# Jack-Tattershall/mujoco-manip

Measured on AMD Instinct MI355X. Metric: env steps/sec (whole node) at 4096 parallel envs; 1/2/4/8 MI355X scaling, higher is better.
Workload: dtype f32

## Files before the change

mujoco_manip_amd/_build.py:

```python
from __future__ import annotations

import os
import subprocess
from concurrent.futures import ThreadPoolExecutor

PKG = os.path.dirname(os.path.abspath(__file__))
CSRC = os.path.join(PKG, "csrc")
LIB = os.path.join(PKG, "libmmx.so")
LIB_PROF = os.path.join(PKG, "libmmx_prof.so")
SOURCES = ["mmx_kernels.hip", "mmx_step_l192.hip", "mmx_render.hip", "mmx_render_lit.hip", "mmx_png.hip",
           "mmx_snapshot.hip", "mmx_mppi.hip", "mmx_policy.hip", "mmx_api.cpp"]
ARCH = os.environ.get("MMX_OFFLOAD_ARCH", "gfx950")
DEVICE_MATH = ["-Xarch_device", "-freciprocal-math", "-Xarch_device", "-fapprox-func",
               "-Xarch_device", "-ffinite-math-only", "-Xarch_device", "-fno-signed-zeros"]
DEVICE_SCHED = ["-mllvm", "-amdgpu-sched-strategy=" + os.environ.get("MMX_SCHED", "iterative-ilp")]
if os.environ.get("MMX_SCHED") == "default":
    DEVICE_SCHED = []
DEVICE_NOSLP = ["-Xarch_device", "-fno-slp-vectorize"]
FLAGS = DEVICE_MATH + DEVICE_SCHED + DEVICE_NOSLP + os.environ.get("MMX_EXTRA_FLAGS", "").split()
SOURCE_FLAGS = {"mmx_kernels.hip": ["-Xarch_device", "-fassociative-math"],
                "mmx_step_l192.hip": ["-Xarch_device", "-fassociative-math"],
                "mmx_mppi.hip": ["-Xarch_device", "-fno-finite-math-only"]}


STEP_SOURCES = ["mmx_kernels.hip", "mmx_step_l192.hip"]
HIPCC_JOBS = 16
TEST_VARIANTS = {
    "libmmx_col4.so": ["MMX_COL_LIST=4", "MMX_CAND_CAP=4"],
    "libmmx_nolist.so": ["MMX_CAND_CAP=1"],
    "libmmx_nocache.so": ["MMX_GJK_CACHE=0", "MMX_PROBE=15"],
    "libmmx_gjkprobe.so": ["MMX_PROBE=15"],
    "libmmx_hdelay.so": ["MMX_HELPER_DELAY=1", "MMX_PROBE=14"],
    "libmmx_edelay.so": ["MMX_HELPER_DELAY=2", "MMX_PROBE=14"],
    "libmmx_synth.so": ["MMX_BUDGET_SYNTH=1"],
}


def lib_path(profile: bool = False) -> str:
    return LIB_PROF if profile else LIB


def test_variant(name: str) -> str:
    path = os.path.join(PKG, name)
    if not os.path.exists(path):
        raise RuntimeError("test build missing: run __graft_entry__.build()")
    return path


def _stale(lib: str) -> bool:
    if not os.path.exists(lib):
        return True
    t = os.path.getmtime(lib)
    inc = os.path.join(PKG, "..", "include")
    deps = [os.path.join(CSRC, f) for f in os.listdir(CSRC) if f.endswith((".hip", ".cpp", ".h", ".inc"))]
    deps += [os.path.join(inc, f) for f in os.listdir(inc) if f.endswith(".h")]
    return any(os.path.getmtime(d) > t for d in deps)


def _hipcc(src: str, obj: str, defines: list[str] | tuple = (), profile: bool = False, verbose: bool = False) -> str:
    cmd = [os.environ.get("HIPCC", "/opt/rocm/bin/hipcc")] + (["-xhip"] if src.endswith(".cpp") else [])
    cmd += FLAGS + SOURCE_FLAGS.get(src, []) + [f"-D{d}" for d in defines] + (["-DMMX_PHASE_CLOCK=1"] if profile else [])
    cmd += [f"--offload-arch={ARCH}", "-O3", "-std=c++17", "-fPIC", "-c", os.path.join(CSRC, src), "-o", obj]
    if verbose:
        print(" ".join(cmd), flush=True)
    subprocess.check_call(cmd)
    return obj

# ... 43 lines not shown
```

mujoco_manip_amd/csrc/mmx_model_gen.h:

```cpp
#ifndef MMX_MODEL_GEN_H
#define MMX_MODEL_GEN_H

#ifndef MMX_MODEL_QUAL
#define MMX_MODEL_QUAL static const
#endif

#define MMX_NBODY 19
#define MMX_NJNT 12
#define MMX_NQ 30
#define MMX_NV 27
#define MMX_NGEOM 47
#define MMX_NMESH 12
#define MMX_NPAIR 780
#define MMX_NU 8
#define MMX_NCAM 3

MMX_MODEL_QUAL int MMX_body_parent[19] = {-1, 0, 1, 2, 3, 4, 5, 6, 7, 8, 9, 9, 0, 0, 0, 0, 0, 0, 0};
MMX_MODEL_QUAL int MMX_body_weld[19] = {0, 0, 2, 3, 4, 5, 6, 7, 8, 8, 10, 11, 0, 0, 0, 0, 16, 17, 18};
MMX_MODEL_QUAL int MMX_body_jnt[19] = {-1, -1, 0, 1, 2, 3, 4, 5, 6, -1, 7, 8, -1, -1, -1, -1, 9, 10, 11};
MMX_MODEL_QUAL float MMX_body_pos[57] = {0.0f, 0.0f, 0.0f, 0.0f, 0.0f, 0.0f, 0.0f, 0.0f, 0.3330000042915344f, 0.0f, 0.0f, 0.0f, 0.0f, -0.3160000145435333f, 0.0f, 0.08250000327825546f, 0.0f, 0.0f, -0.08250000327825546f, 0.3840000033378601f, 0.0f, 0.0f, 0.0f, 0.0f, 0.08799999952316284f, 0.0f, 0.0f, 0.0f, 0.0f, 0.10700000077486038f, 0.0f, 0.0f, 0.058400001376867294f, 0.0f, 0.0f, 0.058400001376867294f, 0.0f, 0.44999998807907104f, 0.0f, -0.30000001192092896f, 0.550000011920929f, 0.23999999463558197f, 0.0f, 0.6499999761581421f, 0.23999999463558197f, 0.30000001192092896f, 0.550000011920929f, 0.23999999463558197f, -0.15000000596046448f, 0.44999998807907104f, 0.25999999046325684f, 0.0f, 0.44999998807907104f, 0.25999999046325684f, 0.15000000596046448f, 0.44999998807907104f, 0.25999999046325684f};
MMX_MODEL_QUAL float MMX_body_quat[76] = {1.0f, 0.0f, 0.0f, 0.0f, 1.0f, 0.0f, 0.0f, 0.0f, 1.0f, 0.0f, 0.0f, 0.0f, 0.7071067690849304f, -0.7071067690849304f, 0.0f, 0.0f, 0.7071067690849304f, 0.7071067690849304f, 0.0f, 0.0f, 0.7071067690849304f, 0.7071067690849304f, 0.0f, 0.0f, 0.7071067690849304f, -0.7071067690849304f, 0.0f, 0.0f, 0.7071067690849304f, 0.7071067690849304f, 0.0f, 0.0f, 0.7071067690849304f, 0.7071067690849304f, 0.0f, 0.0f, 0.9238795638084412f, 0.0f, 0.0f, -0.3826834261417389f, 1.0f, 0.0f, 0.0f, 0.0f, 0.0f, 0.0f, 0.0f, 1.0f, 1.0f, 0.0f, 0.0f, 0.0f, 1.0f, 0.0f, 0.0f, 0.0f, 1.0f, 0.0f, 0.0f, 0.0f, 1.0f, 0.0f, 0.0f, 0.0f, 1.0f, 0.0f, 0.0f, 0.0f, 1.0f, 0.0f, 0.0f, 0.0f, 1.0f, 0.0f, 0.0f, 0.0f};
MMX_MODEL_QUAL float MMX_body_mass[19] = {0.0f, 0.6297690272331238f, 4.970684051513672f, 0.6469259858131409f, 3.2286040782928467f, 3.587894916534424f, 1.2259459495544434f, 1.6665550470352173f, 0.7355219721794128f, 0.7300000190734863f, 0.014999999664723873f, 0.014999999664723873f, 21.570796966552734f, 0.1728000044822693f, 0.1728000044822693f, 0.1728000044822693f, 0.05000000074505806f, 0.05000000074505806f, 0.05000000074505806f};
MMX_MODEL_QUAL float MMX_body_ipos[57] = {0.0f, 0.0f, 0.0f, -0.04101800173521042f, -0.00014000000373926014f, 0.049973998218774796f, 0.003874999936670065f, 0.0020810000132769346f, -0.04761999845504761f, -0.003140999935567379f, -0.028720000758767128f, 0.003495000069960952f, 0.027518000453710556f, 0.03925200179219246f, -0.06650199741125107f, -0.05316999927163124f, 0.10441900044679642f, 0.02745399996638298f, -0.011952999979257584f, 0.041064999997615814f, -0.038437001407146454f, 0.060148999094963074f, -0.014116999693214893f, -0.010517000220716f, 0.010517000220716f, -0.004251999780535698f, 0.06159700080752373f, -0.009999999776482582f, 0.0f, 0.029999999329447746f, 0.0f, 0.0f, 0.0f, 0.0f, 0.0f, 0.0f, 0.0f, 0.0f, 0.2112615406513214f, 0.0f, 0.0f, 0.019999999552965164f, 0.0f, 0.0f, 0.019999999552965164f, 0.0f, 0.0f, 0.019999999552965164f, 0.0f, 0.0f, 0.0f, 0.0f, 0.0f, 0.0f, 0.0f, 0.0f, 0.0f};
MMX_MODEL_QUAL float MMX_body_inertia[171] = {0.0f, 0.0f, 0.0f, 0.0f, 0.0f, 0.0f, 0.0f, 0.0f, 0.0f, 0.0031500000040978193f, 8.29040004646231e-07f, 0.0001500000071246177f, 8.29040004646231e-07f, 0.0038799999747425318f, 8.229900231526699e-06f, 0.0001500000071246177f, 8.229900231526699e-06f, 0.0042849997989833355f, 0.7033699750900269f, -0.00013899999612476677f, 0.006771999876946211f, -0.00013899999612476677f, 0.7066100239753723f, 0.019169000908732414f, 0.006771999876946211f, 0.019169000908732414f, 0.009116999804973602f, 0.007961999624967575f, -0.003924999851733446f, 0.010254000313580036f, -0.003924999851733446f, 0.028109999373555183f, 0.0007040000054985285f, 0.010254000313580036f, 0.0007040000054985285f, 0.025994999334216118f, 0.03724199905991554f, -0.0047610001638531685f, -0.011396000161767006f, -0.0047610001638531685f, 0.03615500032901764f, -0.012804999947547913f, -0.011396000161767006f, -0.012804999947547913f, 0.010830000042915344f, 0.025853000581264496f, 0.007796000223606825f, -0.00133200001437217f, 0.007796000223606825f, 0.019551999866962433f, 0.008640999905765057f, -0.00133200001437217f, 0.008640999905765057f, 0.02832300029695034f, 0.03554899990558624f, -0.0021170000545680523f, -0.004036999773234129f, -0.0021170000545680523f, 0.02947399951517582f, 0.00022899999748915434f, -0.004036999773234129f, 0.00022899999748915434f, 0.008627000264823437f, 0.001964000053703785f, 0.00010900000052060932f, -0.0011579999700188637f, 0.00010900000052060932f, 0.004354000091552734f, 0.00034100000630132854f, -0.0011579999700188637f, 0.00034100000630132854f, 0.005433000158518553f, 0.012516000308096409f, -0.00042799999937415123f, -0.001196000026538968f, -0.00042799999937415123f, 0.01002699974924326f, -0.0007409999961964786f, -0.001196000026538968f, -0.0007409999961964786f, 0.004815000109374523f, 0.0010000000474974513f, 0.0f, 0.0f, 0.0f, 0.0024999999441206455f, 0.0f, 0.0f, 0.0f, 0.0017000000225380063f, 2.3749998945277184e-06f, 0.0f, 0.0f, 0.0f, 2.3749998945277184e-06f, 0.0f, 0.0f, 0.0f, 7.500000265281415e-07f, 2.3749998945277184e-06f, 0.0f, 0.0f, 0.0f, 2.3749998945277184e-06f, 0.0f, 0.0f, 0.0f, 7.500000265281415e-07f, 0.7272951602935791f, 0.0f, 0.0f, 0.0f, 1.2882095575332642f, 0.0f, 0.0f, 0.0f, 1.9577548503875732f, 0.0004148735897615552f, 0.0f, 0.0f, 0.0f, 0.0004148735897615552f, 0.0f, 0.0f, 0.0f, 0.0006913535762578249f, 0.0004148735897615552f, 0.0f, 0.0f, 0.0f, 0.0004148735897615552f, 0.0f, 0.0f, 0.0f, 0.0006913535762578249f, 0.0004148735897615552f, 0.0f, 0.0f, 0.0f, 0.0004148735897615552f, 0.0f, 0.0f, 0.0f, 0.0006913535762578249f, 1.3333333299669903e-05f, 0.0f, 0.0f, 0.0f, 1.3333333299669903e-05f, 0.0f, 0.0f, 0.0f, 1.3333333299669903e-05f, 1.3333333299669903e-05f, 0.0f, 0.0f, 0.0f, 1.3333333299669903e-05f, 0.0f, 0.0f, 0.0f, 1.3333333299669903e-05f, 1.3333333299669903e-05f, 0.0f, 0.0f, 0.0f, 1.3333333299669903e-05f, 0.0f, 0.0f, 0.0f, 1.3333333299669903e-05f};
// ... 36 lines not shown
MMX_MODEL_QUAL float MMX_act_gain[8] = {4500.0f, 4500.0f, 3500.0f, 3500.0f, 2000.0f, 2000.0f, 2000.0f, 0.01568627543747425f};
MMX_MODEL_QUAL float MMX_act_bias[24] = {0.0f, -4500.0f, -450.0f, 0.0f, -4500.0f, -450.0f, 0.0f, -3500.0f, -350.0f, 0.0f, -3500.0f, -350.0f, 0.0f, -2000.0f, -200.0f, 0.0f, -2000.0f, -200.0f, 0.0f, -2000.0f, -200.0f, 0.0f, -100.0f, -10.0f};
MMX_MODEL_QUAL float MMX_act_ctrlrange[16] = {-2.8973000049591064f, 2.8973000049591064f, -1.7627999782562256f, 1.7627999782562256f, -2.8973000049591064f, 2.8973000049591064f, -3.0717999935150146f, -0.0697999969124794f, -2.8973000049591064f, 2.8973000049591064f, -0.017500000074505806f, 3.752500057220459f, -2.8973000049591064f, 2.8973000049591064f, 0.0f, 255.0f};
MMX_MODEL_QUAL float MMX_act_forcerange[16] = {-87.0f, 87.0f, -87.0f, 87.0f, -87.0f, 87.0f, -87.0f, 87.0f, -12.0f, 12.0f, -12.0f, 12.0f, -12.0f, 12.0f, -100.0f, 100.0f};
MMX_MODEL_QUAL int MMX_tendon_jnt[2] = {7, 8};
MMX_MODEL_QUAL float MMX_tendon_coef[2] = {0.5f, 0.5f};
MMX_MODEL_QUAL int MMX_eq_jnt[2] = {7, 8};
MMX_MODEL_QUAL float MMX_eq_solref[2] = {0.004999999888241291f, 1.0f};
MMX_MODEL_QUAL float MMX_eq_solimp[5] = {0.949999988079071f, 0.9900000095367432f, 0.0010000000474974513f, 0.5f, 2.0f};
MMX_MODEL_QUAL int MMX_cam_body[3] = {0, 0, 9};
MMX_MODEL_QUAL float MMX_cam_pos[9] = {0.0f, 0.0f, 2.0f, 1.2000000476837158f, -0.30000001192092896f, 0.800000011920929f, -0.07000000029802322f, 0.0f, 0.054999999701976776f};
MMX_MODEL_QUAL float MMX_cam_quat[12] = {1.0f, 0.0f, 0.0f, 0.0f, 0.5929035544395447f, 0.3853120505809784f, 0.3853120505809784f, 0.5929035544395447f, -0.061601605266332626f, -0.7044183611869812f, 0.7044183611869812f, 0.061601605266332626f};
MMX_MODEL_QUAL float MMX_cam_fovy[3] = {45.0f, 45.0f, 128.0f};
#define MMX_BODY_HAND 9
#define MMX_BODY_OBJ_RED 16
#define MMX_BODY_OBJ_GREEN 17
#define MMX_BODY_OBJ_BLUE 18
#define MMX_BODY_BIN_RED 13
#define MMX_BODY_BIN_GREEN 14
#define MMX_BODY_BIN_BLUE 15
#define MMX_BODY_TABLE 12
#define MMX_CAM_OVERHEAD 0
#define MMX_CAM_WRIST 2
MMX_MODEL_QUAL int MMX_geom_class[47] = {0, 1, 1, 1, 1, 1, 1, 1, 1, 1, 1, 1, 1, 1, 1, 1, 1, 1, 1, 1, 1, 1, 1, 1, 2, 2, 2, 2, 2, 2, 2, 2, 2, 2, 2, 2, 2, 2, 2, 2, 2, 2, 2, 2, 0, 0, 0};
MMX_MODEL_QUAL float MMX_geom_static_xpos[141] = {0.0f, 0.0f, 0.0f, -0.041255850344896317f, 2.8345499231363647e-05f, 0.06998516619205475f, 0.03709043934941292f, 8.725424413569272e-05f, 0.2644845247268677f, -0.037196315824985504f, -0.013869321905076504f, 0.40099474787712097f, -0.02814285084605217f, -0.015605982393026352f, 0.6186633110046387f, 0.027922509238123894f, 0.06398750096559525f, 0.6869798898696899f, -0.022774716839194298f, 0.2227759212255478f, 0.6771363615989685f, -0.07904047518968582f, 0.29724419116973877f, 0.6512680649757385f, -0.07080242037773132f, 0.3996330499649048f, 0.6165943145751953f, 0.006160127930343151f, 0.45152971148490906f, 0.6238852739334106f, 0.026312898844480515f, 0.4878093898296356f, 0.5252102613449097f, -0.001783691463060677f, 0.48299553990364075f, 0.47784945368766785f, 0.05441174656152725f, 0.4765017330646515f, 0.41279593110084534f, 0.04549825191497803f, 0.4747501313686371f, 0.39537930488586426f, 0.04199604317545891f, 0.4796721637248993f, 0.3893578350543976f, 0.04200046509504318f, 0.46872711181640625f, 0.3904559910297394f, 0.04199603945016861f, 0.4807204306125641f, 0.39980536699295044f, 0.042000461369752884f, 0.46977537870407104f, 0.4009035527706146f, -0.05441524460911751f, 0.4764572083950043f, 0.4128003716468811f, -0.04550173878669739f, 0.4747137427330017f, 0.39538291096687317f, -0.04199953004717827f, 0.4686935544013977f, 0.3904593288898468f, -0.042003948241472244f, 0.47963857650756836f, 0.389361172914505f, -0.04199953377246857f, 0.4697417914867401f, 0.40090689063072205f, -0.04200395196676254f, 0.48068684339523315f, 0.39980870485305786f, 0.0f, 0.44999998807907104f, 0.2199999988079071f, 0.3499999940395355f, 0.699999988079071f, 0.10000000149011612f, -0.3499999940395355f, 0.699999988079071f, 0.10000000149011612f, 0.3499999940395355f, 0.20000000298023224f, 0.10000000149011612f, -0.3499999940395355f, 0.20000000298023224f, 0.10000000149011612f, -0.30000001192092896f, 0.550000011920929f, 0.23999999463558197f, -0.30000001192092896f, 0.49000000953674316f, 0.27000001072883606f, -0.30000001192092896f, 0.6100000143051147f, 0.27000001072883606f, -0.36000001430511475f, 0.550000011920929f, 0.27000001072883606f, -0.23999999463558197f, 0.550000011920929f, 0.27000001072883606f, 0.0f, 0.6499999761581421f, 0.23999999463558197f, 0.0f, 0.5899999737739563f, 0.27000001072883606f, 0.0f, 0.7099999785423279f, 0.27000001072883606f, -0.05999999865889549f, 0.6499999761581421f, 0.27000001072883606f, 0.05999999865889549f, 0.6499999761581421f, 0.27000001072883606f, 0.30000001192092896f, 0.550000011920929f, 0.23999999463558197f, 0.30000001192092896f, 0.49000000953674316f, 0.27000001072883606f, 0.30000001192092896f, 0.6100000143051147f, 0.27000001072883606f, 0.23999999463558197f, 0.550000011920929f, 0.27000001072883606f, 0.36000001430511475f, 0.550000011920929f, 0.27000001072883606f, -0.15000000596046448f, 0.44999998807907104f, 0.25999999046325684f, 0.0f, 0.44999998807907104f, 0.25999999046325684f, 0.15000000596046448f, 0.44999998807907104f, 0.25999999046325684f};
MMX_MODEL_QUAL float MMX_geom_static_xmat[423] = {1.0f, 0.0f, 0.0f, 0.0f, 1.0f, 0.0f, 0.0f, 0.0f, 1.0f, 1.0f, 0.0f, 0.0f, 0.0f, 1.0f, 0.0f, 0.0f, 0.0f, 1.0f, -3.6732051285071066e-06f, -1.0f, 0.0f, 1.0f, -3.6732051285071066e-06f, 0.0f, 0.0f, 0.0f, 1.0f, -3.5999855754198506e-06f, -7.297531965377857e-07f, -1.0f, 0.9800665974617004f, 0.19866932928562164f, -3.6732051285071066e-06f, 0.19866932928562164f, -0.9800665974617004f, -2.220444858110231e-16f, -3.5999855754198506e-06f, -1.0f, 7.297531965377857e-07f, 0.9800665974617004f, -3.6732051285071066e-06f, -0.19866932928562164f, 0.19866932928562164f, -4.4259853774201345e-18f, 0.9800665974617004f, 1.1875089285240392e-06f, -3.4759543723339448e-06f, 1.0f, -0.32328957319259644f, 0.9463000893592834f, 3.6732051285071066e-06f, -0.9463000893592834f, -0.32328957319259644f, -2.1319223712349701e-16f, 1.1875089285240392e-06f, -1.0f, -3.4759543723339448e-06f, -0.32328957319259644f, -3.6732051285071066e-06f, 0.9463000893592834f, -0.9463000893592834f, 2.849769559143189e-16f, -0.32328957319259644f, 1.1875089285240392e-06f, -1.0f, -3.4759543723339448e-06f, -0.32328957319259644f, -3.6732051285071066e-06f, 0.9463000893592834f, -0.9463000893592834f, 2.849769559143189e-16f, -0.32328957319259644f, 1.1875089285240392e-06f, -1.0f, -3.4759543723339448e-06f, -0.32328957319259644f, -3.6732051285071066e-06f, 0.9463000893592834f, -0.9463000893592834f, 2.849769559143189e-16f, -0.32328957319259644f, -3.6548544812831096e-06f, -3.6670860481535783e-07f, 1.0f, 0.9950041770935059f, 0.0998334139585495f, 3.6732051285071066e-06f, -0.0998334139585495f, 0.9950041770935059f, -2.131920253652602e-16f, 0.7068225741386414f, 0.7073908448219299f, 3.6670860481535783e-07f, 0.703856885433197f, -0.7032914161682129f, -0.0998334139585495f, -0.07062099128961563f, 0.07056476920843124f, -0.9950041770935059f, -0.0004017833271063864f, 0.9999999403953552f, 3.6670860481535783e-07f, 0.9950040578842163f, 0.00039981267764233053f, -0.0998334139585495f, -0.0998334065079689f, -3.97465264541097e-05f, -0.9950041770935059f, -0.0004017833271063864f, 0.9999999403953552f, 3.6670860481535783e-07f, 0.9950040578842163f, 0.00039981267764233053f, -0.0998334139585495f, -0.0998334065079689f, -3.97465264541097e-05f, -0.9950041770935059f, -0.0004017833271063864f, 0.9999999403953552f, 3.6670860481535783e-07f, 0.9950040578842163f, 0.00039981267764233053f, -0.0998334139585495f, -0.0998334065079689f, -3.97465264541097e-05f, -0.9950041770935059f, -0.0004017833271063864f, 0.9999999403953552f, 3.6670860481535783e-07f, 0.9950040578842163f, 0.00039981267764233053f, -0.0998334139585495f, -0.0998334065079689f, -3.97465264541097e-05f, -0.9950041770935059f, -0.0004017833271063864f, 0.9999999403953552f, 3.6670860481535783e-07f, 0.9950040578842163f, 0.00039981267764233053f, -0.0998334139585495f, -0.0998334065079689f, -3.97465264541097e-05f, -0.9950041770935059f, -0.0004017833271063864f, 0.9999999403953552f, 3.6670860481535783e-07f, 0.9950040578842163f, 0.00039981267764233053f, -0.0998334139585495f, -0.0998334065079689f, -3.97465264541097e-05f, -0.9950041770935059f, -0.0004017833271063864f, 0.9999999403953552f, 3.6670860481535783e-07f, 0.9950040578842163f, 0.00039981267764233053f, -0.0998334139585495f, -0.0998334065079689f, -3.97465264541097e-05f, -0.9950041770935059f, 0.0004017833271063864f, -0.9999999403953552f, 3.6670860481535783e-07f, -0.9950040578842163f, -0.00039981267764233053f, -0.0998334139585495f, 0.0998334065079689f, 3.97465264541097e-05f, -0.9950041770935059f, 0.0004017833271063864f, -0.9999999403953552f, 3.6670860481535783e-07f, -0.9950040578842163f, -0.00039981267764233053f, -0.0998334139585495f, 0.0998334065079689f, 3.97465264541097e-05f, -0.9950041770935059f, 0.0004017833271063864f, -0.9999999403953552f, 3.6670860481535783e-07f, -0.9950040578842163f, -0.00039981267764233053f, -0.0998334139585495f, 0.0998334065079689f, 3.97465264541097e-05f, -0.9950041770935059f, 0.0004017833271063864f, -0.9999999403953552f, 3.6670860481535783e-07f, -0.9950040578842163f, -0.00039981267764233053f, -0.0998334139585495f, 0.0998334065079689f, 3.97465264541097e-05f, -0.9950041770935059f, 0.0004017833271063864f, -0.9999999403953552f, 3.6670860481535783e-07f, -0.9950040578842163f, -0.00039981267764233053f, -0.0998334139585495f, 0.0998334065079689f, 3.97465264541097e-05f, -0.9950041770935059f, 0.0004017833271063864f, -0.9999999403953552f, 3.6670860481535783e-07f, -0.9950040578842163f, -0.00039981267764233053f, -0.0998334139585495f, 0.0998334065079689f, 3.97465264541097e-05f, -0.9950041770935059f, 1.0f, 0.0f, 0.0f, 0.0f, 1.0f, 0.0f, 0.0f, 0.0f, 1.0f, 1.0f, 0.0f, 0.0f, 0.0f, 1.0f, 0.0f, 0.0f, 0.0f, 1.0f, 1.0f, 0.0f, 0.0f, 0.0f, 1.0f, 0.0f, 0.0f, 0.0f, 1.0f, 1.0f, 0.0f, 0.0f, 0.0f, 1.0f, 0.0f, 0.0f, 0.0f, 1.0f, 1.0f, 0.0f, 0.0f, 0.0f, 1.0f, 0.0f, 0.0f, 0.0f, 1.0f, 1.0f, 0.0f, 0.0f, 0.0f, 1.0f, 0.0f, 0.0f, 0.0f, 1.0f, 1.0f, 0.0f, 0.0f, 0.0f, 1.0f, 0.0f, 0.0f, 0.0f, 1.0f, 1.0f, 0.0f, 0.0f, 0.0f, 1.0f, 0.0f, 0.0f, 0.0f, 1.0f, 1.0f, 0.0f, 0.0f, 0.0f, 1.0f, 0.0f, 0.0f, 0.0f, 1.0f, 1.0f, 0.0f, 0.0f, 0.0f, 1.0f, 0.0f, 0.0f, 0.0f, 1.0f, 1.0f, 0.0f, 0.0f, 0.0f, 1.0f, 0.0f, 0.0f, 0.0f, 1.0f, 1.0f, 0.0f, 0.0f, 0.0f, 1.0f, 0.0f, 0.0f, 0.0f, 1.0f, 1.0f, 0.0f, 0.0f, 0.0f, 1.0f, 0.0f, 0.0f, 0.0f, 1.0f, 1.0f, 0.0f, 0.0f, 0.0f, 1.0f, 0.0f, 0.0f, 0.0f, 1.0f, 1.0f, 0.0f, 0.0f, 0.0f, 1.0f, 0.0f, 0.0f, 0.0f, 1.0f, 1.0f, 0.0f, 0.0f, 0.0f, 1.0f, 0.0f, 0.0f, 0.0f, 1.0f, 1.0f, 0.0f, 0.0f, 0.0f, 1.0f, 0.0f, 0.0f, 0.0f, 1.0f, 1.0f, 0.0f, 0.0f, 0.0f, 1.0f, 0.0f, 0.0f, 0.0f, 1.0f, 1.0f, 0.0f, 0.0f, 0.0f, 1.0f, 0.0f, 0.0f, 0.0f, 1.0f, 1.0f, 0.0f, 0.0f, 0.0f, 1.0f, 0.0f, 0.0f, 0.0f, 1.0f, 1.0f, 0.0f, 0.0f, 0.0f, 1.0f, 0.0f, 0.0f, 0.0f, 1.0f, 1.0f, 0.0f, 0.0f, 0.0f, 1.0f, 0.0f, 0.0f, 0.0f, 1.0f, 1.0f, 0.0f, 0.0f, 0.0f, 1.0f, 0.0f, 0.0f, 0.0f, 1.0f};
MMX_MODEL_QUAL float MMX_geom_lmat[423] = {1.0f, 0.0f, 0.0f, 0.0f, 1.0f, 0.0f, 0.0f, 0.0f, 1.0f, 1.0f, 0.0f, 0.0f, 0.0f, 1.0f, 0.0f, 0.0f, 0.0f, 1.0f, 1.0f, 0.0f, 0.0f, 0.0f, 1.0f, 0.0f, 0.0f, 0.0f, 1.0f, 1.0f, 0.0f, 0.0f, 0.0f, 1.0f, 0.0f, 0.0f, 0.0f, 1.0f, 1.0f, 0.0f, 0.0f, 0.0f, 1.0f, 0.0f, 0.0f, 0.0f, 1.0f, 1.0f, 0.0f, 0.0f, 0.0f, 1.0f, 0.0f, 0.0f, 0.0f, 1.0f, 1.0f, 0.0f, 0.0f, 0.0f, 1.0f, 0.0f, 0.0f, 0.0f, 1.0f, 1.0f, 0.0f, 0.0f, 0.0f, 1.0f, 0.0f, 0.0f, 0.0f, 1.0f, 1.0f, 0.0f, 0.0f, 0.0f, 1.0f, 0.0f, 0.0f, 0.0f, 1.0f, 1.0f, 0.0f, 0.0f, 0.0f, 1.0f, 0.0f, 0.0f, 0.0f, 1.0f, 1.0f, 0.0f, 0.0f, 0.0f, 1.0f, 0.0f, 0.0f, 0.0f, 1.0f, 1.0f, 0.0f, 0.0f, 0.0f, 1.0f, 0.0f, 0.0f, 0.0f, 1.0f, 1.0f, 0.0f, 0.0f, 0.0f, 1.0f, 0.0f, 0.0f, 0.0f, 1.0f, 1.0f, 0.0f, 0.0f, 0.0f, 1.0f, 0.0f, 0.0f, 0.0f, 1.0f, 1.0f, 0.0f, 0.0f, 0.0f, 1.0f, 0.0f, 0.0f, 0.0f, 1.0f, 1.0f, 0.0f, 0.0f, 0.0f, 1.0f, 0.0f, 0.0f, 0.0f, 1.0f, 1.0f, 0.0f, 0.0f, 0.0f, 1.0f, 0.0f, 0.0f, 0.0f, 1.0f, 1.0f, 0.0f, 0.0f, 0.0f, 1.0f, 0.0f, 0.0f, 0.0f, 1.0f, 1.0f, 0.0f, 0.0f, 0.0f, 1.0f, 0.0f, 0.0f, 0.0f, 1.0f, 1.0f, 0.0f, 0.0f, 0.0f, 1.0f, 0.0f, 0.0f, 0.0f, 1.0f, 1.0f, 0.0f, 0.0f, 0.0f, 1.0f, 0.0f, 0.0f, 0.0f, 1.0f, 1.0f, 0.0f, 0.0f, 0.0f, 1.0f, 0.0f, 0.0f, 0.0f, 1.0f, 1.0f, 0.0f, 0.0f, 0.0f, 1.0f, 0.0f, 0.0f, 0.0f, 1.0f, 1.0f, 0.0f, 0.0f, 0.0f, 1.0f, 0.0f, 0.0f, 0.0f, 1.0f, 1.0f, 0.0f, 0.0f, 0.0f, 1.0f, 0.0f, 0.0f, 0.0f, 1.0f, 1.0f, 0.0f, 0.0f, 0.0f, 1.0f, 0.0f, 0.0f, 0.0f, 1.0f, 1.0f, 0.0f, 0.0f, 0.0f, 1.0f, 0.0f, 0.0f, 0.0f, 1.0f, 1.0f, 0.0f, 0.0f, 0.0f, 1.0f, 0.0f, 0.0f, 0.0f, 1.0f, 1.0f, 0.0f, 0.0f, 0.0f, 1.0f, 0.0f, 0.0f, 0.0f, 1.0f, 1.0f, 0.0f, 0.0f, 0.0f, 1.0f, 0.0f, 0.0f, 0.0f, 1.0f, 1.0f, 0.0f, 0.0f, 0.0f, 1.0f, 0.0f, 0.0f, 0.0f, 1.0f, 1.0f, 0.0f, 0.0f, 0.0f, 1.0f, 0.0f, 0.0f, 0.0f, 1.0f, 1.0f, 0.0f, 0.0f, 0.0f, 1.0f, 0.0f, 0.0f, 0.0f, 1.0f, 1.0f, 0.0f, 0.0f, 0.0f, 1.0f, 0.0f, 0.0f, 0.0f, 1.0f, 1.0f, 0.0f, 0.0f, 0.0f, 1.0f, 0.0f, 0.0f, 0.0f, 1.0f, 1.0f, 0.0f, 0.0f, 0.0f, 1.0f, 0.0f, 0.0f, 0.0f, 1.0f, 1.0f, 0.0f, 0.0f, 0.0f, 1.0f, 0.0f, 0.0f, 0.0f, 1.0f, 1.0f, 0.0f, 0.0f, 0.0f, 1.0f, 0.0f, 0.0f, 0.0f, 1.0f, 1.0f, 0.0f, 0.0f, 0.0f, 1.0f, 0.0f, 0.0f, 0.0f, 1.0f, 1.0f, 0.0f, 0.0f, 0.0f, 1.0f, 0.0f, 0.0f, 0.0f, 1.0f, 1.0f, 0.0f, 0.0f, 0.0f, 1.0f, 0.0f, 0.0f, 0.0f, 1.0f, 1.0f, 0.0f, 0.0f, 0.0f, 1.0f, 0.0f, 0.0f, 0.0f, 1.0f, 1.0f, 0.0f, 0.0f, 0.0f, 1.0f, 0.0f, 0.0f, 0.0f, 1.0f, 1.0f, 0.0f, 0.0f, 0.0f, 1.0f, 0.0f, 0.0f, 0.0f, 1.0f, 1.0f, 0.0f, 0.0f, 0.0f, 1.0f, 0.0f, 0.0f, 0.0f, 1.0f, 1.0f, 0.0f, 0.0f, 0.0f, 1.0f, 0.0f, 0.0f, 0.0f, 1.0f, 1.0f, 0.0f, 0.0f, 0.0f, 1.0f, 0.0f, 0.0f, 0.0f, 1.0f};
MMX_MODEL_QUAL int MMX_body_static[19] = {1, 1, 0, 0, 0, 0, 0, 0, 0, 0, 0, 0, 1, 1, 1, 1, 0, 0, 0};
MMX_MODEL_QUAL float MMX_body_bsphere[76] = {0.0f, 0.0f, 0.0f, 0.0f, -0.041255850344896317f, 2.8345499231363647e-05f, 0.06998516619205475f, 0.135495126247406f, 8.711800182936713e-05f, -0.03709043934941292f, -0.06851548701524734f, 0.15415802597999573f, -8.425299893133342e-05f, -0.06939476728439331f, 0.037196364253759384f, 0.15506279468536377f, 0.04145773500204086f, 0.028142908588051796f, -0.03293054923415184f, 0.1373220980167389f, -0.041233666241168976f, 0.034429881721735f, 0.027922743931412697f, 0.13788986206054688f, -0.0007534790202043951f, 0.03911004960536957f, -0.11334440857172012f, 0.18793441355228424f, 0.042101308703422546f, 0.015146210789680481f, 0.006161786615848541f, 0.11200033128261566f, 0.018635770305991173f, 0.018578847870230675f, 0.07941387593746185f, 0.08063489943742752f, -1.0067499715660233e-05f, -0.0017819214845076203f, 0.020018674433231354f, 0.10924399644136429f, 4.999999987376214e-07f, 0.01441350020468235f, 0.026995500549674034f, 0.03231212869286537f, 4.999999987376214e-07f, 0.01441350020468235f, 0.026995500549674034f, 0.03231212869286537f, 0.0f, 0.44999998807907104f, 0.2199999988079071f, 0.5496199131011963f, -0.30000001192092896f, 0.550000011920929f, 0.2461177259683609f, 0.13169018924236298f, 0.0f, 0.6499999761581421f, 0.2461177259683609f, 0.13169018924236298f, 0.30000001192092896f, 0.550000011920929f, 0.2461177259683609f, 0.13169018924236298f, 0.0f, 0.0f, 0.0f, 0.03464101627469063f, 0.0f, 0.0f, 0.0f, 0.03464101627469063f, 0.0f, 0.0f, 0.0f, 0.03464101627469063f};
#define MMX_NBODYPAIR 143
MMX_MODEL_QUAL int MMX_bodypair[572] = {0, 2, 0, 1, 0, 3, 1, 1, 0, 4, 2, 1, 0, 5, 3, 1, 0, 6, 4, 3, 0, 7, 7, 1, 0, 8, 8, 1, 0, 9, 9, 1, 0, 10, 10, 6, 0, 11, 16, 6, 0, 16, 22, 1, 0, 17, 23, 1, 0, 18, 24, 1, 1, 3, 25, 1, 1, 4, 26, 1, 1, 5, 27, 1, 1, 6, 28, 3, 1, 7, 31, 1, 1, 8, 32, 1, 1, 9, 33, 1, 1, 10, 34, 6, 1, 11, 40, 6, 1, 16, 46, 1, 1, 17, 47, 1, 1, 18, 48, 1, 2, 4, 49, 1, 2, 5, 50, 1, 2, 6, 51, 3, 2, 7, 54, 1, 2, 8, 55, 1, 2, 9, 56, 1, 2, 10, 57, 6, 2, 11, 63, 6, 2, 12, 69, 5, 2, 13, 74, 5, 2, 14, 79, 5, 2, 15, 84, 5, 2, 16, 89, 1, 2, 17, 90, 1, 2, 18, 91, 1, 3, 5, 92, 1, 3, 6, 93, 3, 3, 7, 96, 1, 3, 8, 97, 1, 3, 9, 98, 1, 3, 10, 99, 6, 3, 11, 105, 6, 3, 12, 111, 5, 3, 13, 116, 5, 3, 14, 121, 5, 3, 15, 126, 5, 3, 16, 131, 1, 3, 17, 132, 1, 3, 18, 133, 1, 4, 6, 134, 3, 4, 7, 137, 1, 4, 8, 138, 1, 4, 9, 139, 1, 4, 10, 140, 6, 4, 11, 146, 6, 4, 12, 152, 5, 4, 13, 157, 5, 4, 14, 162, 5, 4, 15, 167, 5, 4, 16, 172, 1, 4, 17, 173, 1, 4, 18, 174, 1, 5, 7, 175, 1, 5, 8, 176, 1, 5, 9, 177, 1, 5, 10, 178, 6, 5, 11, 184, 6, 5, 12, 190, 5, 5, 13, 195, 5, 5, 14, 200, 5, 5, 15, 205, 5, 5, 16, 210, 1, 5, 17, 211, 1, 5, 18, 212, 1, 6, 8, 213, 3, 6, 9, 216, 3, 6, 10, 219, 18, 6, 11, 237, 18, 6, 12, 255, 15, 6, 13, 270, 15, 6, 14, 285, 15, 6, 15, 300, 15, 6, 16, 315, 3, 6, 17, 318, 3, 6, 18, 321, 3, 7, 10, 324, 6, 7, 11, 330, 6, 7, 12, 336, 5, 7, 13, 341, 5, 7, 14, 346, 5, 7, 15, 351, 5, 7, 16, 356, 1, 7, 17, 357, 1, 7, 18, 358, 1, 8, 12, 359, 5, 8, 13, 364, 5, 8, 14, 369, 5, 8, 15, 374, 5, 8, 16, 379, 1, 8, 17, 380, 1, 8, 18, 381, 1, 9, 12, 382, 5, 9, 13, 387, 5, 9, 14, 392, 5, 9, 15, 397, 5, 9, 16, 402, 1, 9, 17, 403, 1, 9, 18, 404, 1, 10, 11, 405, 36, 10, 12, 441, 30, 10, 13, 471, 30, 10, 14, 501, 30, 10, 15, 531, 30, 10, 16, 561, 6, 10, 17, 567, 6, 10, 18, 573, 6, 11, 12, 579, 30, 11, 13, 609, 30, 11, 14, 639, 30, 11, 15, 669, 30, 11, 16, 699, 6, 11, 17, 705, 6, 11, 18, 711, 6, 12, 16, 717, 5, 12, 17, 722, 5, 12, 18, 727, 5, 13, 16, 732, 5, 13, 17, 737, 5, 13, 18, 742, 5, 14, 16, 747, 5, 14, 17, 752, 5, 14, 18, 757, 5, 15, 16, 762, 5, 15, 17, 767, 5, 15, 18, 772, 5, 16, 17, 777, 1, 16, 18, 778, 1, 17, 18, 779, 1};
MMX_MODEL_QUAL int MMX_bodypair_geoms[1560] = {0, 2, 0, 3, 0, 4, 0, 5, 0, 6, 0, 7, 0, 8, 0, 9, 0, 10, 0, 11, 0, 12, 0, 13, 0, 14, 0, 15, 0, 16, 0, 17, 0, 18, 0, 19, 0, 20, 0, 21, 0, 22, 0, 23, 0, 44, 0, 45, 0, 46, 1, 3, 1, 4, 1, 5, 1, 6, 1, 7, 1, 8, 1, 9, 1, 10, 1, 11, 1, 12, 1, 13, 1, 14, 1, 15, 1, 16, 1, 17, 1, 18, 1, 19, 1, 20, 1, 21, 1, 22, 1, 23, 1, 44, 1, 45, 1, 46, 2, 4, 2, 5, 2, 6, 2, 7, 2, 8, 2, 9, 2, 10, 2, 11, 2, 12, 2, 13, 2, 14, 2, 15, 2, 16, 2, 17, 2, 18, 2, 19, 2, 20, 2, 21, 2, 22, 2, 23, 2, 24, 2, 25, 2, 26, 2, 27, 2, 28, 2, 29, 2, 30, 2, 31, 2, 32, 2, 33, 2, 34, 2, 35, 2, 36, 2, 37, 2, 38, 2, 39, 2, 40, 2, 41, 2, 42, 2, 43, 2, 44, 2, 45, 2, 46, 3, 5, 3, 6, 3, 7, 3, 8, 3, 9, 3, 10, 3, 11, 3, 12, 3, 13, 3, 14, 3, 15, 3, 16, 3, 17, 3, 18, 3, 19, 3, 20, 3, 21, 3, 22, 3, 23, 3, 24, 3, 25, 3, 26, 3, 27, 3, 28, 3, 29, 3, 30, 3, 31, 3, 32, 3, 33, 3, 34, 3, 35, 3, 36, 3, 37, 3, 38, 3, 39, 3, 40, 3, 41, 3, 42, 3, 43, 3, 44, 3, 45, 3, 46, 4, 6, 4, 7, 4, 8, 4, 9, 4, 10, 4, 11, 4, 12, 4, 13, 4, 14, 4, 15, 4, 16, 4, 17, 4, 18, 4, 19, 4, 20, 4, 21, 4, 22, 4, 23, 4, 24, 4, 25, 4, 26, 4, 27, 4, 28, 4, 29, 4, 30, 4, 31, 4, 32, 4, 33, 4, 34, 4, 35, 4, 36, 4, 37, 4, 38, 4, 39, 4, 40, 4, 41, 4, 42, 4, 43, 4, 44, 4, 45, 4, 46, 5, 9, 5, 10, 5, 11, 5, 12, 5, 13, 5, 14, 5, 15, 5, 16, 5, 17, 5, 18, 5, 19, 5, 20, 5, 21, 5, 22, 5, 23, 5, 24, 5, 25, 5, 26, 5, 27, 5, 28, 5, 29, 5, 30, 5, 31, 5, 32, 5, 33, 5, 34, 5, 35, 5, 36, 5, 37, 5, 38, 5, 39, 5, 40, 5, 41, 5, 42, 5, 43, 5, 44, 5, 45, 5, 46, 6, 10, 7, 10, 8, 10, 6, 11, 7, 11, 8, 11, 6, 12, 6, 13, 6, 14, 6, 15, 6, 16, 6, 17, 7, 12, 7, 13, 7, 14, 7, 15, 7, 16, 7, 17, 8, 12, 8, 13, 8, 14, 8, 15, 8, 16, 8, 17, 6, 18, 6, 19, 6, 20, 6, 21, 6, 22, 6, 23, 7, 18, 7, 19, 7, 20, 7, 21, 7, 22, 7, 23, 8, 18, 8, 19, 8, 20, 8, 21, 8, 22, 8, 23, 6, 24, 6, 25, 6, 26, 6, 27, 6, 28, 7, 24, 7, 25, 7, 26, 7, 27, 7, 28, 8, 24, 8, 25, 8, 26, 8, 27, 8, 28, 6, 29, 6, 30, 6, 31, 6, 32, 6, 33, 7, 29, 7, 30, 7, 31, 7, 32, 7, 33, 8, 29, 8, 30, 8, 31, 8, 32, 8, 33, 6, 34, 6, 35, 6, 36, 6, 37, 6, 38, 7, 34, 7, 35, 7, 36, 7, 37, 7, 38, 8, 34, 8, 35, 8, 36, 8, 37, 8, 38, 6, 39, 6, 40, 6, 41, 6, 42, 6, 43, 7, 39, 7, 40, 7, 41, 7, 42, 7, 43, 8, 39, 8, 40, 8, 41, 8, 42, 8, 43, 6, 44, 7, 44, 8, 44, 6, 45, 7, 45, 8, 45, 6, 46, 7, 46, 8, 46, 9, 12, 9, 13, 9, 14, 9, 15, 9, 16, 9, 17, 9, 18, 9, 19, 9, 20, 9, 21, 9, 22, 9, 23, 9, 24, 9, 25, 9, 26, 9, 27, 9, 28, 9, 29, 9, 30, 9, 31, 9, 32, 9, 33, 9, 34, 9, 35, 9, 36, 9, 37, 9, 38, 9, 39, 9, 40, 9, 41, 9, 42, 9, 43, 9, 44, 9, 45, 9, 46, 10, 24, 10, 25, 10, 26, 10, 27, 10, 28, 10, 29, 10, 30, 10, 31, 10, 32, 10, 33, 10, 34, 10, 35, 10, 36, 10, 37, 10, 38, 10, 39, 10, 40, 10, 41, 10, 42, 10, 43, 10, 44, 10, 45, 10, 46, 11, 24, 11, 25, 11, 26, 11, 27, 11, 28, 11, 29, 11, 30, 11, 31, 11, 32, 11, 33, 11, 34, 11, 35, 11, 36, 11, 37, 11, 38, 11, 39, 11, 40, 11, 41, 11, 42, 11, 43, 11, 44, 11, 45, 11, 46, 12, 18, 12, 19, 12, 20, 12, 21, 12, 22, 12, 23, 13, 18, 13, 19, 13, 20, 13, 21, 13, 22, 13, 23, 14, 18, 14, 19, 14, 20, 14, 21, 14, 22, 14, 23, 15, 18, 15, 19, 15, 20, 15, 21, 15, 22, 15, 23, 16, 18, 16, 19, 16, 20, 16, 21, 16, 22, 16, 23, 17, 18, 17, 19, 17, 20, 17, 21, 17, 22, 17, 23, 12, 24, 12, 25, 12, 26, 12, 27, 12, 28, 13, 24, 13, 25, 13, 26, 13, 27, 13, 28, 14, 24, 14, 25, 14, 26, 14, 27, 14, 28, 15, 24, 15, 25, 15, 26, 15, 27, 15, 28, 16, 24, 16, 25, 16, 26, 16, 27, 16, 28, 17, 24, 17, 25, 17, 26, 17, 27, 17, 28, 12, 29, 12, 30, 12, 31, 12, 32, 12, 33, 13, 29, 13, 30, 13, 31, 13, 32, 13, 33, 14, 29, 14, 30, 14, 31, 14, 32, 14, 33, 15, 29, 15, 30, 15, 31, 15, 32, 15, 33, 16, 29, 16, 30, 16, 31, 16, 32, 16, 33, 17, 29, 17, 30, 17, 31, 17, 32, 17, 33, 12, 34, 12, 35, 12, 36, 12, 37, 12, 38, 13, 34, 13, 35, 13, 36, 13, 37, 13, 38, 14, 34, 14, 35, 14, 36, 14, 37, 14, 38, 15, 34, 15, 35, 15, 36, 15, 37, 15, 38, 16, 34, 16, 35, 16, 36, 16, 37, 16, 38, 17, 34, 17, 35, 17, 36, 17, 37, 17, 38, 12, 39, 12, 40, 12, 41, 12, 42, 12, 43, 13, 39, 13, 40, 13, 41, 13, 42, 13, 43, 14, 39, 14, 40, 14, 41, 14, 42, 14, 43, 15, 39, 15, 40, 15, 41, 15, 42, 15, 43, 16, 39, 16, 40, 16, 41, 16, 42, 16, 43, 17, 39, 17, 40, 17, 41, 17, 42, 17, 43, 12, 44, 13, 44, 14, 44, 15, 44, 16, 44, 17, 44, 12, 45, 13, 45, 14, 45, 15, 45, 16, 45, 17, 45, 12, 46, 13, 46, 14, 46, 15, 46, 16, 46, 17, 46, 18, 24, 18, 25, 18, 26, 18, 27, 18, 28, 19, 24, 19, 25, 19, 26, 19, 27, 19, 28, 20, 24, 20, 25, 20, 26, 20, 27, 20, 28, 21, 24, 21, 25, 21, 26, 21, 27, 21, 28, 22, 24, 22, 25, 22, 26, 22, 27, 22, 28, 23, 24, 23, 25, 23, 26, 23, 27, 23, 28, 18, 29, 18, 30, 18, 31, 18, 32, 18, 33, 19, 29, 19, 30, 19, 31, 19, 32, 19, 33, 20, 29, 20, 30, 20, 31, 20, 32, 20, 33, 21, 29, 21, 30, 21, 31, 21, 32, 21, 33, 22, 29, 22, 30, 22, 31, 22, 32, 22, 33, 23, 29, 23, 30, 23, 31, 23, 32, 23, 33, 18, 34, 18, 35, 18, 36, 18, 37, 18, 38, 19, 34, 19, 35, 19, 36, 19, 37, 19, 38, 20, 34, 20, 35, 20, 36, 20, 37, 20, 38, 21, 34, 21, 35, 21, 36, 21, 37, 21, 38, 22, 34, 22, 35, 22, 36, 22, 37, 22, 38, 23, 34, 23, 35, 23, 36, 23, 37, 23, 38, 18, 39, 18, 40, 18, 41, 18, 42, 18, 43, 19, 39, 19, 40, 19, 41, 19, 42, 19, 43, 20, 39, 20, 40, 20, 41, 20, 42, 20, 43, 21, 39, 21, 40, 21, 41, 21, 42, 21, 43, 22, 39, 22, 40, 22, 41, 22, 42, 22, 43, 23, 39, 23, 40, 23, 41, 23, 42, 23, 43, 18, 44, 19, 44, 20, 44, 21, 44, 22, 44, 23, 44, 18, 45, 19, 45, 20, 45, 21, 45, 22, 45, 23, 45, 18, 46, 19, 46, 20, 46, 21, 46, 22, 46, 23, 46, 24, 44, 25, 44, 26, 44, 27, 44, 28, 44, 24, 45, 25, 45, 26, 45, 27, 45, 28, 45, 24, 46, 25, 46, 26, 46, 27, 46, 28, 46, 29, 44, 30, 44, 31, 44, 32, 44, 33, 44, 29, 45, 30, 45, 31, 45, 32, 45, 33, 45, 29, 46, 30, 46, 31, 46, 32, 46, 33, 46, 34, 44, 35, 44, 36, 44, 37, 44, 38, 44, 34, 45, 35, 45, 36, 45, 37, 45, 38, 45, 34, 46, 35, 46, 36, 46, 37, 46, 38, 46, 39, 44, 40, 44, 41, 44, 42, 44, 43, 44, 39, 45, 40, 45, 41, 45, 42, 45, 43, 45, 39, 46, 40, 46, 41, 46, 42, 46, 43, 46, 44, 45, 44, 46, 45, 46};
MMX_MODEL_QUAL int MMX_pair_packed[780] = {512, 768, 1024, 1280, 1536, 1792, 2048, 2304, 2560, 2816, 3072, 3328, 3584, 3840, 4096, 4352, 4608, 4864, 5120, 5376, 5632, 5888, 11264, 11520, 11776, 769, 1025, 1281, 1537, 1793, 2049, 2305, 2561, 2817, 3073, 269, 270, 271, 272, 273, 4609, 275, 276, 277, 278, 279, 300, 301, 302, 1026, 1282, 1538, 1794, 2050, 2306, 2562, 2818, 3074, 525, 526, 527, 528, 529, 4610, 531, 532, 533, 534, 535, 536, 537, 538, 539, 540, 541, 542, 543, 544, 545, 546, 547, 548, 549, 550, 551, 552, 553, 554, 555, 556, 557, 558, 1283, 1539, 1795, 2051, 2307, 2563, 2819, 3075, 781, 782, 783, 784, 785, 4611, 787, 788, 789, 790, 791, 792, 793, 794, 795, 796, 797, 798, 799, 800, 801, 802, 803, 804, 805, 806, 807, 808, 809, 810, 811, 812, 813, 814, 1540, 1796, 2052, 2308, 2564, 2820, 3076, 1037, 1038, 1039, 1040, 1041, 4612, 1043, 1044, 1045, 1046, 1047, 1048, 1049, 1050, 1051, 1052, 1053, 1054, 1055, 1056, 1057, 1058, 1059, 1060, 1061, 1062, 1063, 1064, 1065, 1066, 1067, 1068, 1069, 1070, 2309, 2565, 2821, 3077, 1293, 1294, 1295, 1296, 1297, 4613, 1299, 1300, 1301, 1302, 1303, 1304, 1305, 1306, 1307, 1308, 1309, 1310, 1311, 1312, 1313, 1314, 1315, 1316, 1317, 1318, 1319, 1320, 1321, 1322, 1323, 1324, 1325, 1326, 2566, 2567, 2568, 2822, 2823, 2824, 3078, 1549, 1550, 1551, 1552, 1553, 3079, 1805, 1806, 1807, 1808, 1809, 3080, 2061, 2062, 2063, 2064, 2065, 4614, 1555, 1556, 1557, 1558, 1559, 4615, 1811, 1812, 1813, 1814, 1815, 4616, 2067, 2068, 2069, 2070, 2071, 1560, 1561, 1562, 1563, 1564, 1816, 1817, 1818, 1819, 1820, 2072, 2073, 2074, 2075, 2076, 1565, 1566, 1567, 1568, 1569, 1821, 1822, 1823, 1824, 1825, 2077, 2078, 2079, 2080, 2081, 1570, 1571, 1572, 1573, 1574, 1826, 1827, 1828, 1829, 1830, 2082, 2083, 2084, 2085, 2086, 1575, 1576, 1577, 1578, 1579, 1831, 1832, 1833, 1834, 1835, 2087, 2088, 2089, 2090, 2091, 1580, 1836, 2092, 1581, 1837, 2093, 1582, 1838, 2094, 3081, 2317, 2318, 2319, 2320, 2321, 4617, 2323, 2324, 2325, 2326, 2327, 2328, 2329, 2330, 2331, 2332, 2333, 2334, 2335, 2336, 2337, 2338, 2339, 2340, 2341, 2342, 2343, 2344, 2345, 2346, 2347, 2348, 2349, 2350, 2584, 2585, 2586, 2587, 2588, 2589, 2590, 2591, 2592, 2593, 2594, 2595, 2596, 2597, 2598, 2599, 2600, 2601, 2602, 2603, 2604, 2605, 2606, 2840, 2841, 2842, 2843, 2844, 2845, 2846, 2847, 2848, 2849, 2850, 2851, 2852, 2853, 2854, 2855, 2856, 2857, 2858, 2859, 2860, 2861, 2862, 4620, 3091, 3092, 3093, 3094, 3095, 4621, 4877, 5133, 5389, 5645, 5901, 4622, 4878, 5134, 5390, 5646, 5902, 4623, 4879, 5135, 5391, 5647, 5903, 4624, 4880, 5136, 5392, 5648, 5904, 4625, 4881, 5137, 5393, 5649, 5905, 3096, 3097, 3098, 3099, 3100, 6157, 3353, 3354, 3355, 3356, 6158, 3609, 3610, 3611, 3612, 6159, 3865, 3866, 3867, 3868, 6160, 4121, 4122, 4123, 4124, 6161, 4377, 4378, 4379, 4380, 3101, 3102, 3103, 3104, 3105, 7437, 7693, 7949, 8205, 8461, 7438, 7694, 7950, 8206, 8462, 7439, 7695, 7951, 8207, 8463, 7440, 7696, 7952, 8208, 8464, 7441, 7697, 7953, 8209, 8465, 3106, 3107, 3108, 3109, 3110, 8717, 8973, 9229, 9485, 9741, 8718, 8974, 9230, 9486, 9742, 8719, 8975, 9231, 9487, 9743, 8720, 8976, 9232, 9488, 9744, 8721, 8977, 9233, 9489, 9745, 3111, 3112, 3113, 3114, 3115, 9997, 10253, 10509, 10765, 11021, 9998, 10254, 10510, 10766, 11022, 9999, 10255, 10511, 10767, 11023, 10000, 10256, 10512, 10768, 11024, 10001, 10257, 10513, 10769, 11025, 3116, 11277, 11278, 11279, 11280, 11281, 3117, 11533, 11534, 11535, 11536, 11537, 3118, 11789, 11790, 11791, 11792, 11793, 4632, 4633, 4634, 4635, 4636, 6163, 4889, 4890, 4891, 4892, 6164, 5145, 5146, 5147, 5148, 6165, 5401, 5402, 5403, 5404, 6166, 5657, 5658, 5659, 5660, 6167, 5913, 5914, 5915, 5916, 4637, 4638, 4639, 4640, 4641, 7443, 7699, 7955, 8211, 8467, 7444, 7700, 7956, 8212, 8468, 7445, 7701, 7957, 8213, 8469, 7446, 7702, 7958, 8214, 8470, 7447, 7703, 7959, 8215, 8471, 4642, 4643, 4644, 4645, 4646, 8723, 8979, 9235, 9491, 9747, 8724, 8980, 9236, 9492, 9748, 8725, 8981, 9237, 9493, 9749, 8726, 8982, 9238, 9494, 9750, 8727, 8983, 9239, 9495, 9751, 4647, 4648, 4649, 4650, 4651, 10003, 10259, 10515, 10771, 11027, 10004, 10260, 10516, 10772, 11028, 10005, 10261, 10517, 10773, 11029, 10006, 10262, 10518, 10774, 11030, 10007, 10263, 10519, 10775, 11031, 4652, 11283, 11284, 11285, 11286, 11287, 4653, 11539, 11540, 11541, 11542, 11543, 4654, 11795, 11796, 11797, 11798, 11799, 11288, 11289, 11290, 11291, 11292, 11544, 11545, 11546, 11547, 11548, 11800, 11801, 11802, 11803, 11804, 11293, 11294, 11295, 11296, 11297, 11549, 11550, 11551, 11552, 11553, 11805, 11806, 11807, 11808, 11809, 11298, 11299, 11300, 11301, 11302, 11554, 11555, 11556, 11557, 11558, 11810, 11811, 11812, 11813, 11814, 11303, 11304, 11305, 11306, 11307, 11559, 11560, 11561, 11562, 11563, 11815, 11816, 11817, 11818, 11819, 11564, 11820, 11821};

#define MMX_TIMESTEP 0.002
#define MMX_GRAVITY_Z (-9.81)

#endif
```

mujoco_manip_amd/csrc/mmx_step_collision.inc:

```
DEV Geom geom_pose(const EnvSh& E, int g) {
  Geom G;
  G.g = g;
  G.type = MMX_geom_type[g];
  const int b = MMX_geom_body[g];
  if (MMX_body_static[b]) {
    G.x = V3{MMX_geom_static_xpos[3 * g], MMX_geom_static_xpos[3 * g + 1], MMX_geom_static_xpos[3 * g + 2]};
#pragma unroll
    for (int k = 0; k < 9; k++) G.R.m[k] = MMX_geom_static_xmat[9 * g + k];
  } else {
    const V3 bx = body_x(E, b);
    const M3 bR = body_R(E, b);
    G.x = bx + mul(bR, V3{MMX_geom_pos[3 * g], MMX_geom_pos[3 * g + 1], MMX_geom_pos[3 * g + 2]});
    M3 Lm;
#pragma unroll
    for (int k = 0; k < 9; k++) Lm.m[k] = MMX_geom_lmat[9 * g + k];
    G.R = mul(bR, Lm);
  }
  return G;
}

struct WaveSink {
  EnvSh* E;
  int key;
  bool store;
// ... 65 lines not shown
DEV float list_disp_next(const EnvSh& E, float arm) {
#pragma clang fp reassociate(off) contract(off)
  float s = arm;
  if (LANE >= 10 && LANE < 13) {
    const float* v = E.qvel + 9 + 6 * (LANE - 10);
    s = fmaf(sqrtf(fmaf(v[3], v[3], fmaf(v[4], v[4], v[5] * v[5]))), E.crad,
             sqrtf(fmaf(v[0], v[0], fmaf(v[1], v[1], v[2] * v[2]))));
  }
  return E.cdisp + fmaf(1.25f * 2.f * kDt, wave_max(s), 1e-5f);
}

DEV void collide_prune(EnvSh& E, bool only_ro) {
  float* stats = E.stats;
  CLK_DECL;
  if (LANE == 0) {
    E.ncon = 0;
    E.flags &= ~SHF_ROBOT_OBST;
  }
  float* scr = scr_of(E);
  float* gx = scr + COL_GX;
  int* cand = reinterpret_cast<int*>(scr + COL_CAND);
  bool use_list = false;
  if (!only_ro && E.ncand >= 0) {
#if MMX_STEP_HELPER
    const float nd = list_disp_next(E, arm_body_speed(E));
#else
    const float nd = list_disp_next(E, LANE < 10 ? E.cspd : 0.f);
#endif
    use_list = nd < 0.5f * MMX_CAND_MARGIN;
    SYNC();
    if (LANE == 0 && use_list) E.cdisp = nd;
  }
  const bool rebuild = !only_ro && !use_list;
  if (LANE < MMX_NGEOM) {
    const Geom G = geom_pose(E, LANE);
    float* o = gx + GXS * LANE;
    o[0] = G.x.x; o[1] = G.x.y; o[2] = G.x.z;
#pragma unroll
    for (int k = 0; k < 9; k++) o[3 + k] = G.R.m[k];
    o[GX_RB] = MMX_geom_rbound[LANE];
    o[GX_TYPE] = __int_as_float(G.type);
    o[GX_HALF] = MMX_geom_aabb[3 * LANE];
    o[GX_HALF + 1] = MMX_geom_aabb[3 * LANE + 1];
    o[GX_HALF + 2] = MMX_geom_aabb[3 * LANE + 2];
  }
  if (rebuild) {
    float ext = 0.f;
    if (LANE < MMX_NGEOM) {
      const int b = MMX_geom_body[LANE];
      if (!MMX_body_static[b]) ext = norm(V3{gx[GXS * LANE], gx[GXS * LANE + 1], gx[GXS * LANE + 2]} - body_x(E, b)) +
                                     MMX_geom_rbound[LANE];
    }
    ext = wave_max(ext);
    if (LANE == 0) E.crad = ext;
  }
  SYNC();
  PROBE(2, stats, STAT_T_AUX0);
  auto sphere_test = [&](int p, int pk, float infl) {
    const int g1 = pk & 255, g2 = pk >> 8;
    if (only_ro && !robot_obstacle(g1, g2)) return false;
    const float* o1 = gx + GXS * g1;
    const float* o2 = gx + GXS * g2;
    const V3 d = V3{o2[0] - o1[0], o2[1] - o1[1], o2[2] - o1[2]};
    if (__float_as_int(o1[GX_TYPE]) == GT_PLANE) return d.x * o1[5] + d.y * o1[8] + d.z * o1[11] <= o2[GX_RB] + infl;
    const float rb = o1[GX_RB] + o2[GX_RB] + infl;
    return dot(d, d) <= rb * rb;
  };
  int nc = 0;
  if (use_list) {
    const int n = E.ncand;
    constexpr int NLP = (MMX_CAND_CAP + WG - 1) / WG;
    int lp[NLP], lk[NLP];
    const unsigned short* cl = cand_of(E);
    __builtin_amdgcn_fence(__ATOMIC_ACQUIRE, "workgroup");
#pragma unroll
    for (int q = 0; q < NLP; q++) {
      const int k = q * WG + LANE;
      lp[q] = k < n ? (int)cl[k] : 0;
      lk[q] = WG * q < n ? MMX_pair_packed[lp[q]] : 0;
    }
#pragma unroll
    for (int q = 0; q < NLP; q++) {
      if (WG * q >= n) break;
      const int k = q * WG + LANE;
// ... 18 lines not shown
  int ni = 0;
#pragma unroll
  for (int q = 0; q < NPASS; q++) {
    const unsigned long long m = km[q];
    if ((m >> LANE) & 1ull) {
      const int pos = __builtin_amdgcn_mbcnt_hi((unsigned)(m >> 32), __builtin_amdgcn_mbcnt_lo((unsigned)m, 0u));
      if (nc + pos < COL_LIST) cand[nc + pos] = cand_pack(q * WG + LANE, pg[q]);
    }
    nc += __popcll(m);
    if (rebuild) {
      const unsigned long long mi = ki[q];
      const int pos = __builtin_amdgcn_mbcnt_hi((unsigned)(mi >> 32), __builtin_amdgcn_mbcnt_lo((unsigned)mi, 0u));
      if (((mi >> LANE) & 1ull) && ni + pos < MMX_CAND_CAP) cand_of(E)[ni + pos] = (unsigned short)(q * WG + LANE);
      ni += __popcll(mi);
    }
  }
  if (rebuild) {
    __builtin_amdgcn_fence(__ATOMIC_SEQ_CST, "workgroup");
    if (LANE == 0) {
      E.ncand = ni <= MMX_CAND_CAP ? ni : -1;
      E.cdisp = 0.f;
    }
  }
  if (nc > COL_LIST) {
    if (LANE == 0) E.flags |= SHF_CON_OVF;
    nc = COL_LIST;
  }
  }
  SYNC();
  PROBE(2, stats, STAT_T_AUX1);
  constexpr int NCP = (COL_LIST + WG - 1) / WG;
  int ce[NCP];
  int ncls[3] = {0, 0, 0};
#pragma unroll
  for (int q = 0; q < NCP; q++) {
    const int k = q * WG + LANE;
    int c = 3, p = 0;
    if (q * WG < nc) {
      if (k < nc) {
        p = cand[k];
        int pp, g1, g2;
        cand_unpack(p, pp, g1, g2);
        const Geom A = geom_lds(gx, g1), B = geom_lds(gx, g2);
        if (A.type == GT_PLANE) c = 0;
        else if (obb_overlap(A, B, geom_half(gx, g1), geom_half(gx, g2))) c = (A.type == GT_BOX && B.type == GT_BOX) ? 1 : 2;
      }
#pragma unroll
      for (int t = 0; t < 3; t++) ncls[t] += __popcll(__ballot(c == t));
    }
    ce[q] = p | (c << 24);
  }
  SYNC();
  int base[3] = {0, ncls[0], ncls[0] + ncls[1]};
#pragma unroll
  for (int q = 0; q < NCP; q++) {
    if (q * WG < nc) {
      const int c = ce[q] >> 24;
#pragma unroll
      for (int t = 0; t < 3; t++) base[t] = wave_compact(c == t, cand, base[t], ce[q] & 0xFFFFFF);
    }
  }
  if (LANE == 0) {
    E.ncls[0] = ncls[0];
    E.ncls[1] = ncls[1];
    E.ncls[2] = ncls[2];
  }
  SYNC();
  if (MMX_PROBE == 4 && LANE == 0) {
    stats[STAT_T_AUX0] += (float)nc;
    stats[STAT_T_AUX1] += (float)ncls[1];
    stats[STAT_T_AUX2] += (float)ncls[2];
    stats[STAT_T_AUX3] += (float)ncls[0];
  }
  if (MMX_PROBE == 13 && LANE == 0 && !only_ro) {
    stats[STAT_T_AUX0] += use_list ? 0.f : 1.f;
    stats[STAT_T_AUX1] += (rebuild && E.ncand < 0) ? 1.f : 0.f;
    stats[STAT_T_AUX2] += (float)ncls[1];
    stats[STAT_T_AUX3] += (float)ncls[2];
  }
  if (MMX_PROBE == 14 && LANE == 0 && !only_ro) {
    stats[STAT_T_AUX0] += use_list ? 0.f : 1.f;
    stats[STAT_T_AUX1] = E.cdisp;
  }
  if (MMX_PROBE == 16 && LANE == 0 && !only_ro) {
    stats[STAT_T_AUX0] = fmaxf(stats[STAT_T_AUX0], (float)ncls[2]);
    stats[STAT_T_AUX1] += ncls[2] > 2 ? 1.f : 0.f;
    stats[STAT_T_AUX2] += ncls[2] > 4 ? 1.f : 0.f;
    stats[STAT_T_AUX3] += ncls[2] > MMX_AXIS_SLOTS ? 1.f : 0.f;
  }
  PROBE(2, stats, STAT_T_AUX2);
  PROBE(5, stats, STAT_T_AUX3);
}

// ... 18 lines not shown
    SYNC();
    PROBE(5, stats, STAT_T_AUX0);
    V3* poly = reinterpret_cast<V3*>(scr + COL_WORK + COL_POLY * (LANE >> 2));
    for (int k0 = 0; k0 < n1; k0 += WG / 4) {
      const int k = k0 + (LANE >> 2);
      if (k < n1) {
        int p, g1, g2;
        cand_unpack(cand[n0 + k], p, g1, g2);
        const Geom A = geom_lds(gx, g1), B = geom_lds(gx, g2);
        WaveSink cs(&E, p, !only_ro, g1, g2);
        box_box_quad(cs, A, B, geom_half(gx, g1), geom_half(gx, g2), poly, poly + 8);
      }
    }
    SYNC();
    PROBE(5, stats, STAT_T_AUX1);
  }
  if (which & 2) {
    for (int k = 0; k < n2; k++) {
      int p, g1, g2;
      cand_unpack(cand[n0 + n1 + k], p, g1, g2);
      const Geom A = geom_lds(gx, g1), B = geom_lds(gx, g2);
      WaveSink cs(&E, p, !only_ro, g1, g2);
      convex_convex(cs, A, B, scr + SCR_EPA, ac, p);
    }
    SYNC();
    PROBE(5, stats, STAT_T_AUX2);
  }
}

DEV void collide_sort(EnvSh& E) {
  float* stats = E.stats;
  CLK_DECL;
  float* scr = scr_of(E);
  const int n = min(E.ncon, MMX_MAXCON);
  float* tmp = scr + COL_WORK;
  int kb = 0, rank = 0;
  if (LANE < n) {
    kb = con_key(crec(E, LANE));
    const int key = kb & 0xFFFF;
    for (int j = 0; j < n; j++) rank += (con_key(crec(E, j)) & 0xFFFF) < key;
#pragma unroll
    for (int f = 0; f < CL_F; f++) tmp[f * MMX_MAXCON + rank] = con_of(E)[f * MMX_MAXCON + LANE];
  }
  SYNC();
  for (int k = LANE; k < MMX_MAXCON * CL_F; k += WG) con_of(E)[k] = tmp[k];
  if (LANE == 0) E.ncon = n;
  SYNC();
  PROBE(5, stats, STAT_T_AUX3);
}

DEV void collide_wave(EnvSh& E, bool only_ro) {
  collide_prune(E, only_ro);
  collide_pairs(E, only_ro, 3);
  if (!only_ro) collide_sort(E);
}
```

mujoco_manip_amd/csrc/mmx_step_constraints.inc:

```
DEV void row_ref(const float* solref, const float* solimp, float pos, float& imp_ratio, float& kid, float& B) {
  const float imp = impedance(solimp, pos);
  const float dmax = fminf(fmaxf(solimp[1], 1e-4f), 0.9999f);
  const float tc = fmaxf(solref[0], 2.f * kDt), dr = solref[1];
  const float K = 1.f / (dmax * dmax * tc * tc * dr * dr);
  B = 2.f / (dmax * tc);
  imp_ratio = (1.f - imp) / imp;
  kid = K * imp * pos;
}
DEV void store_row(EnvSh& E, int row, const float* jv, int hdr, float vel, float imp_ratio, float kid, float B,
                   float diag) {
  const float aref = -B * vel - kid;
  if (row < MMX_LDSEFC) {
#pragma unroll
    for (int q = 0; q < 3; q++)
      *reinterpret_cast<float4*>(E.J[q][row]) = make_float4(jv[4 * q], jv[4 * q + 1], jv[4 * q + 2], jv[4 * q + 3]);
    *reinterpret_cast<float4*>(E.J[3][row]) = make_float4(jv[12], jv[13], jv[14], aref);
  } else {
    float4* Jr = reinterpret_cast<float4*>(ovf_j(E, row));
#pragma unroll
    for (int q = 0; q < 3; q++) Jr[q] = make_float4(jv[4 * q], jv[4 * q + 1], jv[4 * q + 2], jv[4 * q + 3]);
    Jr[3] = make_float4(jv[12], jv[13], jv[14], aref);
  }
  hdr_set(E, row, hdr);
  dset(E, row, 1.f / fmaxf(imp_ratio * diag, 1e-15f));
}

struct ConPar {
  int dim;
  float mu0, mu1, kid, B, idiag;
};
template <class R>
DEV ConPar contact_params(const R& cc) {
  const int g1 = con_g1(cc), g2 = con_g2(cc);
  ConPar P;
  P.dim = max(MMX_geom_condim[g1], MMX_geom_condim[g2]);
  P.mu0 = fmaxf(MMX_geom_friction[3 * g1], MMX_geom_friction[3 * g2]);
  P.mu1 = fmaxf(MMX_geom_friction[3 * g1 + 1], MMX_geom_friction[3 * g2 + 1]);
  float solref[2], solimp[5];
#pragma unroll
  for (int k = 0; k < 2; k++) solref[k] = 0.5f * (MMX_geom_solref[2 * g1 + k] + MMX_geom_solref[2 * g2 + k]);
#pragma unroll
  for (int k = 0; k < 5; k++) solimp[k] = 0.5f * (MMX_geom_solimp[5 * g1 + k] + MMX_geom_solimp[5 * g2 + k]);
  float impr;
  row_ref(solref, solimp, cc[CL_DIST], impr, P.kid, P.B);
  const int b1 = MMX_geom_body[g1], b2 = MMX_geom_body[g2];
  const float tran = MMX_body_invweight0[2 * b1] + MMX_body_invweight0[2 * b2];
  const float it = impr * tran;
  P.idiag = P.dim > 1 ? 2.f * P.mu0 * P.mu0 * (it + P.mu0 * P.mu0 * it) : it;
  return P;
}
DEV V3 contact_t1(V3 n) {
  const V3 y = (n.y < 0.5f && n.y > -0.5f) ? V3{0.f, 1.f, 0.f} : V3{0.f, 0.f, 1.f};
  return normalize(y - n * dot(n, y));
}

DEV float contact_row(EnvSh& E, int row, const CReg& cc, int rr, const ConPar& P) {
  const V3 p = V3{cc[CL_POS], cc[CL_POS + 1], cc[CL_POS + 2]};
  const V3 n = V3{cc[CL_N], cc[CL_N + 1], cc[CL_N + 2]};
  const int b1 = MMX_geom_body[con_g1(cc)], b2 = MMX_geom_body[con_g2(cc)];
  const int dim = P.dim;
  const bool used = rr == 0 || (rr < 3 && dim >= 3) || (rr == 3 && dim >= 4);
  const V3 t1 = contact_t1(n);
  const V3 u = rr == 0 ? n : (rr == 1 ? t1 : (rr == 2 ? cross(n, t1) : V3{0.f, 0.f, 0.f}));
  const V3 w = rr == 3 ? n : V3{0.f, 0.f, 0.f};
  const float idiag = P.idiag;
  const int k1 = body_block(b1), k2 = body_block(b2);
  int rb0 = k1 >= 0 ? k1 : k2, rb1 = (k1 >= 0 && k2 >= 0 && k2 != k1) ? k2 : BLK_NONE;
  if (rb1 != BLK_NONE && rb1 < rb0) {
    const int t = rb0;
    rb0 = rb1;
    rb1 = t;
  }
  const unsigned am1 = anc_mask(b1), am2 = anc_mask(b2);
  float vel = 0.f;
  float arm[9];
  const V3 pu = cross(p, u) + w;
#pragma unroll
  for (int d = 0; d < 9; d++) {
    const float coef = (float)((int)((am2 >> d) & 1u) - (int)((am1 >> d) & 1u));
    const SV sd = load_S(E, d);
    arm[d] = coef * (dot(u, sd.v) + dot(sd.w, pu));
    vel = fmaf(arm[d], E.qvel[d], vel);
  }
  float cubeA[6], cubeB[6];
  float cvs[2][6];
#pragma unroll
  for (int side = 0; side < 2; side++) {
    const int b = side ? b2 : b1, blk = side ? k2 : k1;
#pragma unroll
    for (int j = 0; j < 6; j++) cvs[side][j] = 0.f;
    if (blk > 0) {
      const float sg = side ? 1.f : -1.f;
      const V3 x = body_x(E, b);
      const M3 R = body_R(E, b);
      cvs[side][0] = sg * u.x;
      cvs[side][1] = sg * u.y;
      cvs[side][2] = sg * u.z;
      const V3 ru = cross(p - x, u) + w;
#pragma unroll
      for (int k = 0; k < 3; k++) cvs[side][3 + k] = sg * dot(col(R, k), ru);
      const int d0 = blk_d0(blk);
#pragma unroll
      for (int j = 0; j < 6; j++) vel = fmaf(cvs[side][j], E.qvel[d0 + j], vel);
    }
  }
  const bool swap = k1 != rb0;
#pragma unroll
  for (int j = 0; j < 6; j++) {
    cubeA[j] = swap ? cvs[1][j] : cvs[0][j];
    cubeB[j] = swap ? cvs[0][j] : cvs[1][j];
  }
  float jv[16];
  const bool armrow = rb0 == 0;
#pragma unroll
  for (int j = 0; j < 16; j++) {
    const float va = j < 9 ? arm[j] : (j < 15 ? cubeB[j - 9] : 0.f);
    const float vc = j < 6 ? cubeA[j] : (j < 12 ? cubeB[j - 6] : 0.f);
    jv[j] = armrow ? va : vc;
  }
  store_row(E, row, jv, rb0 | (rb1 << 4), vel, 1.f, rr == 0 ? P.kid : 0.f, P.B, idiag);
  if (!used) dset(E, row, 0.f);
  return !used || rr == 0 ? (rr == 0 ? 0.f : -1.f) : (rr < 3 ? P.mu0 : P.mu1);
}

DEV void make_constraints_wave(EnvSh& E, float* mu_out) {
  float* stats = E.stats;
  CLK_DECL;
  const float def_ref[2] = {0.02f, 1.0f};
  const float def_imp[5] = {0.9f, 0.95f, 0.001f, 0.5f, 2.0f};
  const int ncon = E.ncon;
  CReg own;
#pragma unroll
  for (int k = 0; k < CL_F; k++) own.v[k] = LANE < ncon ? crec(E, LANE)[k] : 0.f;
  auto rowmap_set = [&](int r, int m) { dset(E, r, __int_as_float(m)); };
  int nlim = 0, tc = -1, nedge = 0;
  bool lo_act = false, hi_act = false;
  if (LANE < 9) {
    const float q = E.qpos[LANE];
    lo_act = q - MMX_jnt_range[2 * LANE] < 0.f;
    hi_act = MMX_jnt_range[2 * LANE + 1] - q < 0.f;
    nlim = (int)lo_act + (int)hi_act;
  }
  if (LANE < ncon) {
    const int g1 = con_g1(own), g2 = con_g2(own);
    const int dim = max(MMX_geom_condim[g1], MMX_geom_condim[g2]);
    nedge = dim == 1 ? 1 : 2 * (dim - 1);
    const int k1 = body_block(MMX_geom_body[g1]), k2 = body_block(MMX_geom_body[g2]);
    int rb0 = k1 >= 0 ? k1 : k2, rb1 = (k1 >= 0 && k2 >= 0 && k2 != k1) ? k2 : BLK_NONE;
    if (rb1 != BLK_NONE && rb1 < rb0) {
      const int t = rb0;
      rb0 = rb1;
      rb1 = t;
    }
    tc = row_type(rb0, rb1);
  }
  const int acnt = (LANE == 0 ? 1 : 0) + nlim;
  const unsigned long long a0 = __ballot(acnt & 1), a1 = __ballot(acnt & 2);
  const int nsingle_raw = __popcll(a0) + 2 * __popcll(a1);
  const int arow = (int)__builtin_amdgcn_mbcnt_hi((unsigned)(a0 >> 32), __builtin_amdgcn_mbcnt_lo((unsigned)a0, 0u)) +
                   2 * (int)__builtin_amdgcn_mbcnt_hi((unsigned)(a1 >> 32), __builtin_amdgcn_mbcnt_lo((unsigned)a1, 0u));
  const int nsingle = (nsingle_raw + 3) & ~3;
  int brow = 0, base = 0;
#pragma unroll
  for (int t = 0; t < NTYPE; t++) {
    const unsigned long long m = __ballot(tc == t);
    const int first = base + (t == 0 ? nsingle : 0);
    if (tc == t) brow = first + 4 * (int)__builtin_amdgcn_mbcnt_hi((unsigned)(m >> 32), __builtin_amdgcn_mbcnt_lo((unsigned)m, 0u));
    if (LANE == 0) E.tbase[t] = min(base, MMX_MAXEFC);
    base = first + 4 * __popcll(m);
  }
  const int total = base;
  const int nefc = min(total, MMX_MAXEFC);
  const int nefc_mj = nsingle_raw + __popcll(__ballot(nedge & 1)) + 2 * __popcll(__ballot(nedge & 2)) +
                      4 * __popcll(__ballot(nedge & 4));
  if (LANE == 0) {
    E.tbase[NTYPE] = nefc;
    E.nefc = nefc;
    E.nefc_mj = nefc_mj;
    E.nsingle = nsingle;
    if (total > MMX_MAXEFC) E.flags |= SHF_EFC_OVF;
  }
  PROBE(3, stats, STAT_T_AUX0);
  if (LANE < 4 && nsingle_raw + LANE < nsingle) rowmap_set(nsingle_raw + LANE, -1);
  int row = arow;
  if (LANE == 0 && row < MMX_MAXEFC) rowmap_set(row++, -1);
  if (LANE < 9) {
#pragma unroll
    for (int side = 0; side < 2; side++)
      if ((side == 0 ? lo_act : hi_act) && row < MMX_MAXEFC) rowmap_set(row++, -1);
  }
  PROBE(3, stats, STAT_T_AUX1);
  ConPar Pc{1, 0.f, 0.f, 0.f, 0.f, 1.f};
  if (LANE < ncon) Pc = contact_params(own);
  if (LANE < ncon) {
#pragma unroll
    for (int rr = 0; rr < 4; rr++)
      if (brow + rr < MMX_MAXEFC) rowmap_set(brow + rr, LANE | (rr << 8));
  }
  ovf_fence(nefc);
  SYNC();
  PROBE(3, stats, STAT_T_AUX3);
  constexpr int RPB = (MMX_MAXEFC + WG - 1) / WG;
  float mu[RPB];
#pragma unroll
  for (int q = 0; q < RPB; q++) {
    const int r = LANE + WG * q;
    mu[q] = 0.f;
    if (WG * q >= nefc) continue;
    const int m = r < nefc ? __float_as_int(dget(E, r)) : -1;
    const int c = m >= 0 ? (m & 255) : 0;
    ConPar P;
    P.dim = __shfl(Pc.dim, c);
    P.mu0 = __shfl(Pc.mu0, c);
    P.mu1 = __shfl(Pc.mu1, c);
    P.kid = __shfl(Pc.kid, c);
    P.B = __shfl(Pc.B, c);
    P.idiag = __shfl(Pc.idiag, c);
    CReg cc;
    cc.v[CL_DIST] = 0.f;
#pragma unroll
    for (int k = CL_POS; k < CL_F; k++) cc.v[k] = __shfl(own.v[k], c);
    if (m >= 0) mu[q] = contact_row(E, r, cc, m >> 8, P);
  }
  row = arow;
  float jv[16];
  if (LANE == 0 && row < MMX_MAXEFC) {
#pragma unroll
    for (int j = 0; j < 16; j++) jv[j] = j == 7 ? 1.f : (j == 8 ? -1.f : 0.f);
    float ir, kid, B;
    row_ref(MMX_eq_solref, MMX_eq_solimp, E.qpos[7] - E.qpos[8], ir, kid, B);
    store_row(E, row, jv, 0 | (BLK_NONE << 4), E.qvel[7] - E.qvel[8], ir, kid, B,
              MMX_dof_invweight0[7] + MMX_dof_invweight0[8]);
    row++;
  }
  if (LANE < 9) {
    const float q = E.qpos[LANE];
#pragma unroll
    for (int side = 0; side < 2; side++) {
      const bool act = side == 0 ? lo_act : hi_act;
      if (act && row < MMX_MAXEFC) {
        const float sg = side == 0 ? 1.f : -1.f;
#pragma unroll
        for (int j = 0; j < 16; j++) jv[j] = j == LANE ? sg : 0.f;
        const float dist = side == 0 ? q - MMX_jnt_range[2 * LANE] : MMX_jnt_range[2 * LANE + 1] - q;
        float ir, kid, B;
        row_ref(def_ref, def_imp, dist, ir, kid, B);
        store_row(E, row, jv, 0 | (BLK_NONE << 4), sg * E.qvel[LANE], ir, kid, B, MMX_dof_invweight0[LANE]);
        row++;
      }
    }
  }
  if (LANE < 4 && nsingle_raw + LANE < nsingle) {
#pragma unroll
    for (int j = 0; j < 16; j++) jv[j] = 0.f;
    store_row(E, nsingle_raw + LANE, jv, 0 | (BLK_NONE << 4), 0.f, 1.f, 0.f, 0.f, 1.f);
// ... 9 lines not shown
```

mujoco_manip_amd/csrc/mmx_step_lds.inc:

```
enum { CL_DIST = 0, CL_POS = 1, CL_N = 4, CL_KEY = 7, CL_F };
static_assert(MMX_NGEOM <= 64 && MMX_NPAIR * 8 < 65536, "contact key packing");
struct CRec {
  const float* b;
  int c;
  DEV float operator[](int k) const { return b[k * MMX_MAXCON + c]; }
};
struct CRecW {
  float* b;
  int c;
  DEV float& operator[](int k) const { return b[k * MMX_MAXCON + c]; }
};
struct CReg {
  float v[CL_F];
  DEV float operator[](int k) const { return v[k]; }
};
template <class R>
DEV int con_key(const R& c) { return __float_as_int(c[CL_KEY]); }
template <class R>
DEV int con_g1(const R& c) { return (con_key(c) >> 16) & 63; }
template <class R>
DEV int con_g2(const R& c) { return (con_key(c) >> 22) & 63; }
#define GST 17
struct EnvSh {
  float qpos[30], qvel[28], ctrl[8];
// ... 61 lines not shown
              "the narrowphase work space exceeds COL_END");
#define SCR_DYN ((COL_END + 3) & ~3)
#define SCR_IKW SCR_DYN
#define SCR_EPA SCR_DYN
#else
#define SCR_DYN COL_WORK
#define SCR_IKW 0
#define SCR_EPA COL_EPA
#endif
#define SCR_IC (SCR_DYN + 272)
#define SCR_AF (SCR_IC + 120)
#define SCR_BIAS (SCR_AF + 8)
#define SCR_OBS COL_WORK
#define SCR_ACT (COL_WORK + 96)
static_assert(SCR_BIAS + 9 <= SCR_FLOATS && SCR_OBS + MMX_NOBS <= SCR_ACT && SCR_ACT + 12 <= SCR_FLOATS &&
                  SCR_EPA + EPA_SCRATCH_FLOATS <= SCR_FLOATS && SCR_IKW + 72 <= SCR_FLOATS,
              "scratch layout");
#ifndef MMX_HELPER_DELAY
#define MMX_HELPER_DELAY 0
#endif
#if MMX_HELPER_DELAY && MMX_STEP_HELPER
#define MMX_DELAY_SLEEPS 4
DEV void delay_wave() {
#pragma unroll
  for (int k = 0; k < MMX_DELAY_SLEEPS; k++) __builtin_amdgcn_s_sleep(127);
  asm volatile("" ::: "memory");
}
#define DELAY_HELPER() do { if (MMX_HELPER_DELAY == 1) delay_wave(); } while (0)
#define DELAY_ENV() do { if (MMX_HELPER_DELAY == 2) delay_wave(); } while (0)
#else
#define DELAY_HELPER() do { } while (0)
#define DELAY_ENV() do { } while (0)
#endif
DEV float* scr_of(EnvSh& E) { return reinterpret_cast<float*>(&E.J); }
DEV const float* scr_of(const EnvSh& E) { return reinterpret_cast<const float*>(&E.J); }
DEV float* obs_of(EnvSh& E) { return scr_of(E) + SCR_OBS; }
DEV const float* obs_of(const EnvSh& E) { return scr_of(E) + SCR_OBS; }
DEV float* con_of(EnvSh& E) { return scr_of(E) + COL_CON; }
DEV CRec crec(const EnvSh& E, int c) { return CRec{scr_of(E) + COL_CON, c}; }
DEV float* lrow_of(EnvSh& E) { return E.G; }
DEV float* arrow_of(EnvSh& E) { return E.ovf + MMX_OVF_ARROW_AT(MMX_LDSEFC); }
DEV unsigned short* cand_of(const EnvSh& E) { return reinterpret_cast<unsigned short*>(E.ovf + MMX_OVF_CAND_AT(MMX_LDSEFC)); }
DEV float* axis_of(const EnvSh& E) { return E.ovf + MMX_OVF_AXIS_AT(MMX_LDSEFC); }
static_assert(MMX_LDSEFC % WG == 0 && MMX_LDSEFC <= MMX_MAXEFC, "LDS rows: whole lane slices");
DEV float* ovf_j(const EnvSh& E, int i) { return E.ovf + 16 * (i - MMX_LDSEFC); }
DEV float* ovf_d(const EnvSh& E, int i) { return E.ovf + 16 * MMX_OVFEFC + (i - MMX_LDSEFC); }
DEV float* ovf_nc(const EnvSh& E, int i) { return E.ovf + 17 * MMX_OVFEFC + (i - MMX_LDSEFC); }
DEV float& jlds(EnvSh& E, int i, int k) { return E.J[k >> 2][i][k & 3]; }
DEV const float& jlds(const EnvSh& E, int i, int k) { return E.J[k >> 2][i][k & 3]; }
DEV float4 jrow4(const EnvSh& E, int i, int q) {
  if (i >= MMX_LDSEFC) return reinterpret_cast<const float4*>(ovf_j(E, i))[q];
  return *reinterpret_cast<const float4*>(E.J[q][i]);
}
DEV float jget(const EnvSh& E, int i, int k) { return i < MMX_LDSEFC ? jlds(E, i, k) : ovf_j(E, i)[k]; }
DEV void jset(EnvSh& E, int i, int k, float v) {
  if (i < MMX_LDSEFC) jlds(E, i, k) = v;
  else ovf_j(E, i)[k] = v;
}
DEV float dget(const EnvSh& E, int i) { return i < MMX_LDSEFC ? E.D[i] : *ovf_d(E, i); }
DEV void dset(EnvSh& E, int i, float v) {
  if (i < MMX_LDSEFC) E.D[i] = v;
  else *ovf_d(E, i) = v;
}
DEV float ncget(const EnvSh& E, int i) { return i < MMX_LDSEFC ? E.NC[i] : *ovf_nc(E, i); }
DEV unsigned char* ovf_hdr(const EnvSh& E) { return reinterpret_cast<unsigned char*>(E.ovf + MMX_OVF_HDR_AT(MMX_LDSEFC)); }
DEV int hdr_get(const EnvSh& E, int i) { return i < MMX_LDSEFC ? E.hdr[i] : ovf_hdr(E)[i - MMX_LDSEFC]; }
// ... 34 lines not shown
  if (k < KIN_HAND_MAT) return E.bx[body_slot(MMX_BODY_HAND)][k - KIN_HAND_POS];
  if (k < KIN_AXIS) return E.bR[body_slot(MMX_BODY_HAND)][k - KIN_HAND_MAT];
  if (k < KIN_ANCHOR) return E.S[(k - KIN_AXIS) / 3][(k - KIN_AXIS) % 3];
  if (k < KIN_OBJ) return E.bx[body_slot(MMX_jnt_body[(k - KIN_ANCHOR) / 3])][(k - KIN_ANCHOR) % 3];
  return E.bx[11 + (k - KIN_OBJ) / 3][(k - KIN_OBJ) % 3];
}
DEV float kin_get(const EnvSh& E, int k) { return kin_ref(const_cast<EnvSh&>(E), k); }
DEV int body_block(int b) { return (b >= 2 && b <= 11) ? 0 : (b >= 16 ? b - 15 : -1); }
#define BLK_NONE 15
DEV int blk_size(int b) { return b == 0 ? 9 : (b == BLK_NONE ? 0 : 6); }
DEV int blk_d0(int b) { return b == 0 ? 0 : 9 + 6 * (b - 1); }
DEV int dof_blk(int a) { return a < 9 ? 0 : 1 + (a - 9) / 6; }
DEV int row_slot(int h, int a) {
  const int b0 = h & 15, b1 = (h >> 4) & 15, ba = dof_blk(a);
  if (ba == b0) return a - blk_d0(b0);
  if (ba == b1) return blk_size(b0) + a - blk_d0(b1);
  return -1;
}
#define NTYPE 10
static constexpr int kTB0[NTYPE] = {0, 0, 0, 0, 1, 1, 1, 2, 2, 3};
static constexpr int kTB1[NTYPE] = {15, 1, 2, 3, 15, 2, 3, 15, 3, 15};
DEV int row_type(int b0, int b1) {
  return b0 == 0 ? (b1 == BLK_NONE ? 0 : b1) : (b0 == 1 ? (b1 == BLK_NONE ? 4 : 3 + b1) : (b0 == 2 ? (b1 == BLK_NONE ? 7 : 8) : 9));
}
DEV bool arm_anc(int d, int b) { return d <= 6 ? (b >= d + 2 && b <= 11) : (d == 7 ? b == 10 : b == 11); }
DEV unsigned anc_mask(int b) {
  return b >= 2 && b <= 11 ? ((1u << min(b - 1, 7)) - 1u) | (b == 10 ? 0x80u : 0u) | (b == 11 ? 0x100u : 0u) : 0u;
}
DEV V3 body_x(const EnvSh& E, int b) {
  if (MMX_body_static[b]) return V3{0.f, 0.f, 0.f};
  const int s = body_slot(b);
  return V3{E.bx[s][0], E.bx[s][1], E.bx[s][2]};
}
DEV M3 body_R(const EnvSh& E, int b) {
  M3 R;
  const int s = body_slot(b);
#pragma unroll
  for (int k = 0; k < 9; k++) R.m[k] = E.bR[s][k];
  return R;
}
DEV SV load_S(const EnvSh& E, int d) { return SV{V3{E.S[d][0], E.S[d][1], E.S[d][2]}, V3{E.S[d][3], E.S[d][4], E.S[d][5]}}; }

template <int CTRL>
DEV float dpp_f(float v) {
  return __int_as_float(__builtin_amdgcn_update_dpp(0, __float_as_int(v), CTRL, 0xF, 0xF, true));
}
DEV float wave_sum(float v) {
  v += dpp_f<0xB1>(v);
  v += dpp_f<0x4E>(v);
  v += dpp_f<0x141>(v);
  v += dpp_f<0x140>(v);
  return (__int_as_float(__builtin_amdgcn_readlane(__float_as_int(v), 0)) +
          __int_as_float(__builtin_amdgcn_readlane(__float_as_int(v), 16))) +
         (__int_as_float(__builtin_amdgcn_readlane(__float_as_int(v), 32)) +
          __int_as_float(__builtin_amdgcn_readlane(__float_as_int(v), 48)));
}
DEV float readlane_max0(float v) { return __int_as_float(__builtin_amdgcn_readlane(__float_as_int(v), 0)); }
DEV float wave_max(float v) {
  v = fmaxf(v, dpp_f<0xB1>(v));
  v = fmaxf(v, dpp_f<0x4E>(v));
  v = fmaxf(v, dpp_f<0x141>(v));
  v = fmaxf(v, dpp_f<0x140>(v));
  return fmaxf(fmaxf(readlane_max0(v), __int_as_float(__builtin_amdgcn_readlane(__float_as_int(v), 16))),
               fmaxf(__int_as_float(__builtin_amdgcn_readlane(__float_as_int(v), 32)),
                     __int_as_float(__builtin_amdgcn_readlane(__float_as_int(v), 48))));
}
// ... 18 lines not shown
```

Baseline: 3.514 million.

## Pack per-geom pose/contact params into aligned tables and skip arm Jacobian when unused

Adds packed, 16-byte-aligned per-geom tables for pose and contact parameters, read with vector int4 loads instead of many scattered constant-array lookups. Contact rows now receive a precomputed body word carrying block ids, ancestor masks and condim, broadcast by shuffle. A wave-wide ballot skips the 9-DOF arm projection when no contact in the wave touches the arm. Collision sorting is also reworked to a rank-based in-place scatter. The old path stays behind MMX_PLAIN_ROWS as a test variant. The new path adds code complexity and a larger constant table, and the skip only pays off when no arm contacts are present.

```diff
diff --git a/mujoco_manip_amd/_build.py b/mujoco_manip_amd/_build.py
--- a/mujoco_manip_amd/_build.py
+++ b/mujoco_manip_amd/_build.py
@@ -33,6 +33,7 @@
     "libmmx_hdelay.so": ["MMX_HELPER_DELAY=1", "MMX_PROBE=14"],
     "libmmx_edelay.so": ["MMX_HELPER_DELAY=2", "MMX_PROBE=14"],
     "libmmx_synth.so": ["MMX_BUDGET_SYNTH=1"],
+    "libmmx_plainrows.so": ["MMX_PLAIN_ROWS=1"],
 }
 
 
diff --git a/mujoco_manip_amd/csrc/mmx_model_gen.h b/mujoco_manip_amd/csrc/mmx_model_gen.h
--- a/mujoco_manip_amd/csrc/mmx_model_gen.h
+++ b/mujoco_manip_amd/csrc/mmx_model_gen.h
@@ -92,6 +92,10 @@
 MMX_MODEL_QUAL int MMX_bodypair[572] = {0, 2, 0, 1, 0, 3, 1, 1, 0, 4, 2, 1, 0, 5, 3, 1, 0, 6, 4, 3, 0, 7, 7, 1, 0, 8, 8, 1, 0, 9, 9, 1, 0, 10, 10, 6, 0, 11, 16, 6, 0, 16, 22, 1, 0, 17, 23, 1, 0, 18, 24, 1, 1, 3, 25, 1, 1, 4, 26, 1, 1, 5, 27, 1, 1, 6, 28, 3, 1, 7, 31, 1, 1, 8, 32, 1, 1, 9, 33, 1, 1, 10, 34, 6, 1, 11, 40, 6, 1, 16, 46, 1, 1, 17, 47, 1, 1, 18, 48, 1, 2, 4, 49, 1, 2, 5, 50, 1, 2, 6, 51, 3, 2, 7, 54, 1, 2, 8, 55, 1, 2, 9, 56, 1, 2, 10, 57, 6, 2, 11, 63, 6, 2, 12, 69, 5, 2, 13, 74, 5, 2, 14, 79, 5, 2, 15, 84, 5, 2, 16, 89, 1, 2, 17, 90, 1, 2, 18, 91, 1, 3, 5, 92, 1, 3, 6, 93, 3, 3, 7, 96, 1, 3, 8, 97, 1, 3, 9, 98, 1, 3, 10, 99, 6, 3, 11, 105, 6, 3, 12, 111, 5, 3, 13, 116, 5, 3, 14, 121, 5, 3, 15, 126, 5, 3, 16, 131, 1, 3, 17, 132, 1, 3, 18, 133, 1, 4, 6, 134, 3, 4, 7, 137, 1, 4, 8, 138, 1, 4, 9, 139, 1, 4, 10, 140, 6, 4, 11, 146, 6, 4, 12, 152, 5, 4, 13, 157, 5, 4, 14, 162, 5, 4, 15, 167, 5, 4, 16, 172, 1, 4, 17, 173, 1, 4, 18, 174, 1, 5, 7, 175, 1, 5, 8, 176, 1, 5, 9, 177, 1, 5, 10, 178, 6, 5, 11, 184, 6, 5, 12, 190, 5, 5, 13, 195, 5, 5, 14, 200, 5, 5, 15, 205, 5, 5, 16, 210, 1, 5, 17, 211, 1, 5, 18, 212, 1, 6, 8, 213, 3, 6, 9, 216, 3, 6, 10, 219, 18, 6, 11, 237, 18, 6, 12, 255, 15, 6, 13, 270, 15, 6, 14, 285, 15, 6, 15, 300, 15, 6, 16, 315, 3, 6, 17, 318, 3, 6, 18, 321, 3, 7, 10, 324, 6, 7, 11, 330, 6, 7, 12, 336, 5, 7, 13, 341, 5, 7, 14, 346, 5, 7, 15, 351, 5, 7, 16, 356, 1, 7, 17, 357, 1, 7, 18, 358, 1, 8, 12, 359, 5, 8, 13, 364, 5, 8, 14, 369, 5, 8, 15, 374, 5, 8, 16, 379, 1, 8, 17, 380, 1, 8, 18, 381, 1, 9, 12, 382, 5, 9, 13, 387, 5, 9, 14, 392, 5, 9, 15, 397, 5, 9, 16, 402, 1, 9, 17, 403, 1, 9, 18, 404, 1, 10, 11, 405, 36, 10, 12, 441, 30, 10, 13, 471, 30, 10, 14, 501, 30, 10, 15, 531, 30, 10, 16, 561, 6, 10, 17, 567, 6, 10, 18, 573, 6, 11, 12, 579, 30, 11, 13, 609, 30, 11, 14, 639, 30, 11, 15, 669, 30, 11, 16, 699, 6, 11, 17, 705, 6, 11, 18, 711, 6, 12, 16, 717, 5, 12, 17, 722, 5, 12, 18, 727, 5, 13, 16, 732, 5, 13, 17, 737, 5, 13, 18, 742, 5, 14, 16, 747, 5, 14, 17, 752, 5, 14, 18, 757, 5, 15, 16, 762, 5, 15, 17, 767, 5, 15, 18, 772, 5, 16, 17, 777, 1, 16, 18, 778, 1, 17, 18, 779, 1};
 MMX_MODEL_QUAL int MMX_bodypair_geoms[1560] = {0, 2, 0, 3, 0, 4, 0, 5, 0, 6, 0, 7, 0, 8, 0, 9, 0, 10, 0, 11, 0, 12, 0, 13, 0, 14, 0, 15, 0, 16, 0, 17, 0, 18, 0, 19, 0, 20, 0, 21, 0, 22, 0, 23, 0, 44, 0, 45, 0, 46, 1, 3, 1, 4, 1, 5, 1, 6, 1, 7, 1, 8, 1, 9, 1, 10, 1, 11, 1, 12, 1, 13, 1, 14, 1, 15, 1, 16, 1, 17, 1, 18, 1, 19, 1, 20, 1, 21, 1, 22, 1, 23, 1, 44, 1, 45, 1, 46, 2, 4, 2, 5, 2, 6, 2, 7, 2, 8, 2, 9, 2, 10, 2, 11, 2, 12, 2, 13, 2, 14, 2, 15, 2, 16, 2, 17, 2, 18, 2, 19, 2, 20, 2, 21, 2, 22, 2, 23, 2, 24, 2, 25, 2, 26, 2, 27, 2, 28, 2, 29, 2, 30, 2, 31, 2, 32, 2, 33, 2, 34, 2, 35, 2, 36, 2, 37, 2, 38, 2, 39, 2, 40, 2, 41, 2, 42, 2, 43, 2, 44, 2, 45, 2, 46, 3, 5, 3, 6, 3, 7, 3, 8, 3, 9, 3, 10, 3, 11, 3, 12, 3, 13, 3, 14, 3, 15, 3, 16, 3, 17, 3, 18, 3, 19, 3, 20, 3, 21, 3, 22, 3, 23, 3, 24, 3, 25, 3, 26, 3, 27, 3, 28, 3, 29, 3, 30, 3, 31, 3, 32, 3, 33, 3, 34, 3, 35, 3, 36, 3, 37, 3, 38, 3, 39, 3, 40, 3, 41, 3, 42, 3, 43, 3, 44, 3, 45, 3, 46, 4, 6, 4, 7, 4, 8, 4, 9, 4, 10, 4, 11, 4, 12, 4, 13, 4, 14, 4, 15, 4, 16, 4, 17, 4, 18, 4, 19, 4, 20, 4, 21, 4, 22, 4, 23, 4, 24, 4, 25, 4, 26, 4, 27, 4, 28, 4, 29, 4, 30, 4, 31, 4, 32, 4, 33, 4, 34, 4, 35, 4, 36, 4, 37, 4, 38, 4, 39, 4, 40, 4, 41, 4, 42, 4, 43, 4, 44, 4, 45, 4, 46, 5, 9, 5, 10, 5, 11, 5, 12, 5, 13, 5, 14, 5, 15, 5, 16, 5, 17, 5, 18, 5, 19, 5, 20, 5, 21, 5, 22, 5, 23, 5, 24, 5, 25, 5, 26, 5, 27, 5, 28, 5, 29, 5, 30, 5, 31, 5, 32, 5, 33, 5, 34, 5, 35, 5, 36, 5, 37, 5, 38, 5, 39, 5, 40, 5, 41, 5, 42, 5, 43, 5, 44, 5, 45, 5, 46, 6, 10, 7, 10, 8, 10, 6, 11, 7, 11, 8, 11, 6, 12, 6, 13, 6, 14, 6, 15, 6, 16, 6, 17, 7, 12, 7, 13, 7, 14, 7, 15, 7, 16, 7, 17, 8, 12, 8, 13, 8, 14, 8, 15, 8, 16, 8, 17, 6, 18, 6, 19, 6, 20, 6, 21, 6, 22, 6, 23, 7, 18, 7, 19, 7, 20, 7, 21, 7, 22, 7, 23, 8, 18, 8, 19, 8, 20, 8, 21, 8, 22, 8, 23, 6, 24, 6, 25, 6, 26, 6, 27, 6, 28, 7, 24, 7, 25, 7, 26, 7, 27, 7, 28, 8, 24, 8, 25, 8, 26, 8, 27, 8, 28, 6, 29, 6, 30, 6, 31, 6, 32, 6, 33, 7, 29, 7, 30, 7, 31, 7, 32, 7, 33, 8, 29, 8, 30, 8, 31, 8, 32, 8, 33, 6, 34, 6, 35, 6, 36, 6, 37, 6, 38, 7, 34, 7, 35, 7, 36, 7, 37, 7, 38, 8, 34, 8, 35, 8, 36, 8, 37, 8, 38, 6, 39, 6, 40, 6, 41, 6, 42, 6, 43, 7, 39, 7, 40, 7, 41, 7, 42, 7, 43, 8, 39, 8, 40, 8, 41, 8, 42, 8, 43, 6, 44, 7, 44, 8, 44, 6, 45, 7, 45, 8, 45, 6, 46, 7, 46, 8, 46, 9, 12, 9, 13, 9, 14, 9, 15, 9, 16, 9, 17, 9, 18, 9, 19, 9, 20, 9, 21, 9, 22, 9, 23, 9, 24, 9, 25, 9, 26, 9, 27, 9, 28, 9, 29, 9, 30, 9, 31, 9, 32, 9, 33, 9, 34, 9, 35, 9, 36, 9, 37, 9, 38, 9, 39, 9, 40, 9, 41, 9, 42, 9, 43, 9, 44, 9, 45, 9, 46, 10, 24, 10, 25, 10, 26, 10, 27, 10, 28, 10, 29, 10, 30, 10, 31, 10, 32, 10, 33, 10, 34, 10, 35, 10, 36, 10, 37, 10, 38, 10, 39, 10, 40, 10, 41, 10, 42, 10, 43, 10, 44, 10, 45, 10, 46, 11, 24, 11, 25, 11, 26, 11, 27, 11, 28, 11, 29, 11, 30, 11, 31, 11, 32, 11, 33, 11, 34, 11, 35, 11, 36, 11, 37, 11, 38, 11, 39, 11, 40, 11, 41, 11, 42, 11, 43, 11, 44, 11, 45, 11, 46, 12, 18, 12, 19, 12, 20, 12, 21, 12, 22, 12, 23, 13, 18, 13, 19, 13, 20, 13, 21, 13, 22, 13, 23, 14, 18, 14, 19, 14, 20, 14, 21, 14, 22, 14, 23, 15, 18, 15, 19, 15, 20, 15, 21, 15, 22, 15, 23, 16, 18, 16, 19, 16, 20, 16, 21, 16, 22, 16, 23, 17, 18, 17, 19, 17, 20, 17, 21, 17, 22, 17, 23, 12, 24, 12, 25, 12, 26, 12, 27, 12, 28, 13, 24, 13, 25, 13, 26, 13, 27, 13, 28, 14, 24, 14, 25, 14, 26, 14, 27, 14, 28, 15, 24, 15, 25, 15, 26, 15, 27, 15, 28, 16, 24, 16, 25, 16, 26, 16, 27, 16, 28, 17, 24, 17, 25, 17, 26, 17, 27, 17, 28, 12, 29, 12, 30, 12, 31, 12, 32, 12, 33, 13, 29, 13, 30, 13, 31, 13, 32, 13, 33, 14, 29, 14, 30, 14, 31, 14, 32, 14, 33, 15, 29, 15, 30, 15, 31, 15, 32, 15, 33, 16, 29, 16, 30, 16, 31, 16, 32, 16, 33, 17, 29, 17, 30, 17, 31, 17, 32, 17, 33, 12, 34, 12, 35, 12, 36, 12, 37, 12, 38, 13, 34, 13, 35, 13, 36, 13, 37, 13, 38, 14, 34, 14, 35, 14, 36, 14, 37, 14, 38, 15, 34, 15, 35, 15, 36, 15, 37, 15, 38, 16, 34, 16, 35, 16, 36, 16, 37, 16, 38, 17, 34, 17, 35, 17, 36, 17, 37, 17, 38, 12, 39, 12, 40, 12, 41, 12, 42, 12, 43, 13, 39, 13, 40, 13, 41, 13, 42, 13, 43, 14, 39, 14, 40, 14, 41, 14, 42, 14, 43, 15, 39, 15, 40, 15, 41, 15, 42, 15, 43, 16, 39, 16, 40, 16, 41, 16, 42, 16, 43, 17, 39, 17, 40, 17, 41, 17, 42, 17, 43, 12, 44, 13, 44, 14, 44, 15, 44, 16, 44, 17, 44, 12, 45, 13, 45, 14, 45, 15, 45, 16, 45, 17, 45, 12, 46, 13, 46, 14, 46, 15, 46, 16, 46, 17, 46, 18, 24, 18, 25, 18, 26, 18, 27, 18, 28, 19, 24, 19, 25, 19, 26, 19, 27, 19, 28, 20, 24, 20, 25, 20, 26, 20, 27, 20, 28, 21, 24, 21, 25, 21, 26, 21, 27, 21, 28, 22, 24, 22, 25, 22, 26, 22, 27, 22, 28, 23, 24, 23, 25, 23, 26, 23, 27, 23, 28, 18, 29, 18, 30, 18, 31, 18, 32, 18, 33, 19, 29, 19, 30, 19, 31, 19, 32, 19, 33, 20, 29, 20, 30, 20, 31, 20, 32, 20, 33, 21, 29, 21, 30, 21, 31, 21, 32, 21, 33, 22, 29, 22, 30, 22, 31, 22, 32, 22, 33, 23, 29, 23, 30, 23, 31, 23, 32, 23, 33, 18, 34, 18, 35, 18, 36, 18, 37, 18, 38, 19, 34, 19, 35, 19, 36, 19, 37, 19, 38, 20, 34, 20, 35, 20, 36, 20, 37, 20, 38, 21, 34, 21, 35, 21, 36, 21, 37, 21, 38, 22, 34, 22, 35, 22, 36, 22, 37, 22, 38, 23, 34, 23, 35, 23, 36, 23, 37, 23, 38, 18, 39, 18, 40, 18, 41, 18, 42, 18, 43, 19, 39, 19, 40, 19, 41, 19, 42, 19, 43, 20, 39, 20, 40, 20, 41, 20, 42, 20, 43, 21, 39, 21, 40, 21, 41, 21, 42, 21, 43, 22, 39, 22, 40, 22, 41, 22, 42, 22, 43, 23, 39, 23, 40, 23, 41, 23, 42, 23, 43, 18, 44, 19, 44, 20, 44, 21, 44, 22, 44, 23, 44, 18, 45, 19, 45, 20, 45, 21, 45, 22, 45, 23, 45, 18, 46, 19, 46, 20, 46, 21, 46, 22, 46, 23, 46, 24, 44, 25, 44, 26, 44, 27, 44, 28, 44, 24, 45, 25, 45, 26, 45, 27, 45, 28, 45, 24, 46, 25, 46, 26, 46, 27, 46, 28, 46, 29, 44, 30, 44, 31, 44, 32, 44, 33, 44, 29, 45, 30, 45, 31, 45, 32, 45, 33, 45, 29, 46, 30, 46, 31, 46, 32, 46, 33, 46, 34, 44, 35, 44, 36, 44, 37, 44, 38, 44, 34, 45, 35, 45, 36, 45, 37, 45, 38, 45, 34, 46, 35, 46, 36, 46, 37, 46, 38, 46, 39, 44, 40, 44, 41, 44, 42, 44, 43, 44, 39, 45, 40, 45, 41, 45, 42, 45, 43, 45, 39, 46, 40, 46, 41, 46, 42, 46, 43, 46, 44, 45, 44, 46, 45, 46};
 MMX_MODEL_QUAL int MMX_pair_packed[780] = {512, 768, 1024, 1280, 1536, 1792, 2048, 2304, 2560, 2816, 3072, 3328, 3584, 3840, 4096, 4352, 4608, 4864, 5120, 5376, 5632, 5888, 11264, 11520, 11776, 769, 1025, 1281, 1537, 1793, 2049, 2305, 2561, 2817, 3073, 269, 270, 271, 272, 273, 4609, 275, 276, 277, 278, 279, 300, 301, 302, 1026, 1282, 1538, 1794, 2050, 2306, 2562, 2818, 3074, 525, 526, 527, 528, 529, 4610, 531, 532, 533, 534, 535, 536, 537, 538, 539, 540, 541, 542, 543, 544, 545, 546, 547, 548, 549, 550, 551, 552, 553, 554, 555, 556, 557, 558, 1283, 1539, 1795, 2051, 2307, 2563, 2819, 3075, 781, 782, 783, 784, 785, 4611, 787, 788, 789, 790, 791, 792, 793, 794, 795, 796, 797, 798, 799, 800, 801, 802, 803, 804, 805, 806, 807, 808, 809, 810, 811, 812, 813, 814, 1540, 1796, 2052, 2308, 2564, 2820, 3076, 1037, 1038, 1039, 1040, 1041, 4612, 1043, 1044, 1045, 1046, 1047, 1048, 1049, 1050, 1051, 1052, 1053, 1054, 1055, 1056, 1057, 1058, 1059, 1060, 1061, 1062, 1063, 1064, 1065, 1066, 1067, 1068, 1069, 1070, 2309, 2565, 2821, 3077, 1293, 1294, 1295, 1296, 1297, 4613, 1299, 1300, 1301, 1302, 1303, 1304, 1305, 1306, 1307, 1308, 1309, 1310, 1311, 1312, 1313, 1314, 1315, 1316, 1317, 1318, 1319, 1320, 1321, 1322, 1323, 1324, 1325, 1326, 2566, 2567, 2568, 2822, 2823, 2824, 3078, 1549, 1550, 1551, 1552, 1553, 3079, 1805, 1806, 1807, 1808, 1809, 3080, 2061, 2062, 2063, 2064, 2065, 4614, 1555, 1556, 1557, 1558, 1559, 4615, 1811, 1812, 1813, 1814, 1815, 4616, 2067, 2068, 2069, 2070, 2071, 1560, 1561, 1562, 1563, 1564, 1816, 1817, 1818, 1819, 1820, 2072, 2073, 2074, 2075, 2076, 1565, 1566, 1567, 1568, 1569, 1821, 1822, 1823, 1824, 1825, 2077, 2078, 2079, 2080, 2081, 1570, 1571, 1572, 1573, 1574, 1826, 1827, 1828, 1829, 1830, 2082, 2083, 2084, 2085, 2086, 1575, 1576, 1577, 1578, 1579, 1831, 1832, 1833, 1834, 1835, 2087, 2088, 2089, 2090, 2091, 1580, 1836, 2092, 1581, 1837, 2093, 1582, 1838, 2094, 3081, 2317, 2318, 2319, 2320, 2321, 4617, 2323, 2324, 2325, 2326, 2327, 2328, 2329, 2330, 2331, 2332, 2333, 2334, 2335, 2336, 2337, 2338, 2339, 2340, 2341, 2342, 2343, 2344, 2345, 2346, 2347, 2348, 2349, 2350, 2584, 2585, 2586, 2587, 2588, 2589, 2590, 2591, 2592, 2593, 2594, 2595, 2596, 2597, 2598, 2599, 2600, 2601, 2602, 2603, 2604, 2605, 2606, 2840, 2841, 2842, 2843, 2844, 2845, 2846, 2847, 2848, 2849, 2850, 2851, 2852, 2853, 2854, 2855, 2856, 2857, 2858, 2859, 2860, 2861, 2862, 4620, 3091, 3092, 3093, 3094, 3095, 4621, 4877, 5133, 5389, 5645, 5901, 4622, 4878, 5134, 5390, 5646, 5902, 4623, 4879, 5135, 5391, 5647, 5903, 4624, 4880, 5136, 5392, 5648, 5904, 4625, 4881, 5137, 5393, 5649, 5905, 3096, 3097, 3098, 3099, 3100, 6157, 3353, 3354, 3355, 3356, 6158, 3609, 3610, 3611, 3612, 6159, 3865, 3866, 3867, 3868, 6160, 4121, 4122, 4123, 4124, 6161, 4377, 4378, 4379, 4380, 3101, 3102, 3103, 3104, 3105, 7437, 7693, 7949, 8205, 8461, 7438, 7694, 7950, 8206, 8462, 7439, 7695, 7951, 8207, 8463, 7440, 7696, 7952, 8208, 8464, 7441, 7697, 7953, 8209, 8465, 3106, 3107, 3108, 3109, 3110, 8717, 8973, 9229, 9485, 9741, 8718, 8974, 9230, 9486, 9742, 8719, 8975, 9231, 9487, 9743, 8720, 8976, 9232, 9488, 9744, 8721, 8977, 9233, 9489, 9745, 3111, 3112, 3113, 3114, 3115, 9997, 10253, 10509, 10765, 11021, 9998, 10254, 10510, 10766, 11022, 9999, 10255, 10511, 10767, 11023, 10000, 10256, 10512, 10768, 11024, 10001, 10257, 10513, 10769, 11025, 3116, 11277, 11278, 11279, 11280, 11281, 3117, 11533, 11534, 11535, 11536, 11537, 3118, 11789, 11790, 11791, 11792, 11793, 4632, 4633, 4634, 4635, 4636, 6163, 4889, 4890, 4891, 4892, 6164, 5145, 5146, 5147, 5148, 6165, 5401, 5402, 5403, 5404, 6166, 5657, 5658, 5659, 5660, 6167, 5913, 5914, 5915, 5916, 4637, 4638, 4639, 4640, 4641, 7443, 7699, 7955, 8211, 8467, 7444, 7700, 7956, 8212, 8468, 7445, 7701, 7957, 8213, 8469, 7446, 7702, 7958, 8214, 8470, 7447, 7703, 7959, 8215, 8471, 4642, 4643, 4644, 4645, 4646, 8723, 8979, 9235, 9491, 9747, 8724, 8980, 9236, 9492, 9748, 8725, 8981, 9237, 9493, 9749, 8726, 8982, 9238, 9494, 9750, 8727, 8983, 9239, 9495, 9751, 4647, 4648, 4649, 4650, 4651, 10003, 10259, 10515, 10771, 11027, 10004, 10260, 10516, 10772, 11028, 10005, 10261, 10517, 10773, 11029, 10006, 10262, 10518, 10774, 11030, 10007, 10263, 10519, 10775, 11031, 4652, 11283, 11284, 11285, 11286, 11287, 4653, 11539, 11540, 11541, 11542, 11543, 4654, 11795, 11796, 11797, 11798, 11799, 11288, 11289, 11290, 11291, 11292, 11544, 11545, 11546, 11547, 11548, 11800, 11801, 11802, 11803, 11804, 11293, 11294, 11295, 11296, 11297, 11549, 11550, 11551, 11552, 11553, 11805, 11806, 11807, 11808, 11809, 11298, 11299, 11300, 11301, 11302, 11554, 11555, 11556, 11557, 11558, 11810, 11811, 11812, 11813, 11814, 11303, 11304, 11305, 11306, 11307, 11559, 11560, 11561, 11562, 11563, 11815, 11816, 11817, 11818, 11819, 11564, 11820, 11821};
+#define MMX_GEOM_POSE_W 20
+#define MMX_GEOM_PAR_W 12
+alignas(16) MMX_MODEL_QUAL int MMX_geom_pose[940] = {0, 0, 1, 0, 1232348160, 1232348160, 0, 0, 0, 0, 1065353216, 0, 0, 0, 1065353216, 0, 0, 0, 1065353216, 0, 7, 1, 1, 1040891708, 1038553002, 1036112822, 1032807788, -1121387547, 938329983, 1032803426, 1065353216, 0, 0, 0, 1065353216, 0, 0, 0, 1065353216, 0, 7, 2, 0, 1042144154, 1029805412, 1035796149, 1039984533, 951497503, -1122505691, -1114877479, 1065353216, 0, 0, 0, 1065353216, 0, 0, 0, 1065353216, 0, 7, 3, 0, 1042204872, 1029804091, 1040135692, 1035797534, -1196379908, -1114759464, 1025006391, 1065353216, 0, 0, 0, 1065353216, 0, 0, 0, 1065353216, 0, 7, 4, 0, 1041014314, 1036308971, 1034558317, 1035233011, 1026150294, 1021742069, -1123622353, 1065353216, 0, 0, 0, 1065353216, 0, 0, 0, 1065353216, 0, 7, 5, 0, 1041052416, 1036345169, 1035433347, 1034567609, -1121393502, 1024263769, 1021623869, 1065353216, 0, 0, 0, 1065353216, 0, 0, 0, 1065353216, 0, 7, 6, 0, 1036890721, 1028900883, 1033452957, 1031848962, -1169849057, 1018859604, -1102523061, 1065353216, 0, 0, 0, 1065353216, 0, 0, 0, 1065353216, 0, 7, 6, 0, 1033724098, 1025534913, 1022017807, 1031022030, -1179185307, 1034018662, -1108330583, 1065353216, 0, 0, 0, 1065353216, 0, 0, 0, 1065353216, 0, 7, 6, 0, 1034022594, 1027688762, 1029785773, 1030773285, -1171822449, 1032912919, -1139367898, 1065353216, 0, 0, 0, 1065353216, 0, 0, 0, 1065353216, 0, 7, 7, 0, 1038442606, 1035504060, 1032340310, 1028482759, 1026323052, 1014507472, 1003088080, 1065353216, 0, 0, 0, 1065353216, 0, 0, 0, 1065353216, 0, 7, 8, 0, 1034232809, 1031821649, 1031813341, 1021355758, 1016637963, 1016607403, 1034068926, 1065353216, 0, 0, 0, 1065353216, 0, 0, 0, 1065353216, 0, 7, 9, 0, 1038072657, 1023511068, 1037128274, 1027354426, -1222056043, -1159098531, 1017380404, 1065353216, 0, 0, 0, 1065353216, 0, 0, 0, 1065353216, 0, 7, 10, 0, 1023357316, 1009520252, 1011055703, 1021054655, 889599933, 1013720730, 1021126059, 1065353216, 0, 0, 0, 1065353216, 0, 0, 0, 1065353216, 0, 6, 10, 0, 1011847436, 1007371158, 998445679, 1007371158, 0, 1001666904, 1026966946, 1065353216, 0, 0, 0, 1065353216, 0, 0, 0, 1065353216, 0, 6, 10, 0, 999928335, 994352038, 990057071, 994352038, 1001666904, 990057071, 1028443341, 1065353216, 0, 0, 0, 1065353216, 0, 0, 0, 1065353216, 0, 6, 10, 0, 999928335, 994352038, 990057071, 994352038, -1145816744, 990057071, 1028443341, 1065353216, 0, 0, 0, 1065353216, 0, 0, 0, 1065353216, 0, 6, 10, 0, 1000646716, 994352038, 990057071, 996499522, 1001666904, 990057071, 1025624769, 1065353216, 0, 0, 0, 1065353216, 0, 0, 0, 1065353216, 0, 6, 10, 0, 1000646716, 994352038, 990057071, 996499522, -1145816744, 990057071, 1025624769, 1065353216, 0, 0, 0, 1065353216, 0, 0, 0, 1065353216, 0, 7, 11, 0, 1023357316, 1009520252, 1011055703, 1021054655, 889599933, 1013720730, 1021126059, 1065353216, 0, 0, 0, 1065353216, 0, 0, 0, 1065353216, 0, 6, 11, 0, 1011847436, 1007371158, 998445679, 1007371158, 0, 1001666904, 1026966946, 1065353216, 0, 0, 0, 1065353216, 0, 0, 0, 1065353216, 0, 6, 11, 0, 999928335, 994352038, 990057071, 994352038, 1001666904, 990057071, 1028443341, 1065353216, 0, 0, 0, 1065353216, 0, 0, 0, 1065353216, 0, 6, 11, 0, 999928335, 994352038, 990057071, 994352038, -1145816744, 990057071, 1028443341, 1065353216, 0, 0, 0, 1065353216, 0, 0, 0, 1065353216, 0, 6, 11, 0, 1000646716, 994352038, 990057071, 996499522, 1001666904, 990057071, 1025624769, 1065353216, 0, 0, 0, 1065353216, 0, 0, 0, 1065353216, 0, 6, 11, 0, 1000646716, 994352038, 990057071, 996499522, -1145816744, 990057071, 1025624769, 1065353216, 0, 0, 0, 1065353216, 0, 0, 0, 1065353216, 0, 6, 12, 1, 1056971316, 1053609165, 1050253722, 1017370378, 0, 1055286886, 1046562734, 1065353216, 0, 0, 0, 1065353216, 0, 0, 0, 1065353216, 0, 5, 12, 1, 1037245023, 1020054733, 1020054733, 1036831949, 1051931443, 1060320051, 1036831949, 1065353216, 0, 0, 0, 1065353216, 0, 0, 0, 1065353216, 0, 5, 12, 1, 1037245023, 1020054733, 1020054733, 1036831949, -1095552205, 1060320051, 1036831949, 1065353216, 0, 0, 0, 1065353216, 0, 0, 0, 1065353216, 0, 5, 12, 1, 1037245023, 1020054733, 1020054733, 1036831949, 1051931443, 1045220557, 1036831949, 1065353216, 0, 0, 0, 1065353216, 0, 0, 0, 1065353216, 0, 5, 12, 1, 1037245023, 1020054733, 1020054733, 1036831949, -1095552205, 1045220557, 1036831949, 1065353216, 0, 0, 0, 1065353216, 0, 0, 0, 1065353216, 0, 6, 13, 1, 1034802091, 1031127695, 1031127695, 990057071, -1097229926, 1057803469, 1047904911, 1065353216, 0, 0, 0, 1065353216, 0, 0, 0, 1065353216, 0, 6, 13, 1, 1032417776, 1031127695, 990057071, 1022739087, -1097229926, 1056629064, 1049247089, 1065353216, 0, 0, 0, 1065353216, 0, 0, 0, 1065353216, 0, 6, 13, 1, 1032417776, 1031127695, 990057071, 1022739087, -1097229926, 1058810102, 1049247089, 1065353216, 0, 0, 0, 1065353216, 0, 0, 0, 1065353216, 0, 6, 13, 1, 1032417776, 990057071, 1031127695, 1022739087, -1095216660, 1057803469, 1049247089, 1065353216, 0, 0, 0, 1065353216, 0, 0, 0, 1065353216, 0, 6, 13, 1, 1032417776, 990057071, 1031127695, 1022739087, -1099578737, 1057803469, 1049247089, 1065353216, 0, 0, 0, 1065353216, 0, 0, 0, 1065353216, 0, 6, 14, 1, 1034802091, 1031127695, 1031127695, 990057071, 0, 1059481190, 1047904911, 1065353216, 0, 0, 0, 1065353216, 0, 0, 0, 1065353216, 0, 6, 14, 1, 1032417776, 1031127695, 990057071, 1022739087, 0, 1058474557, 1049247089, 1065353216, 0, 0, 0, 1065353216, 0, 0, 0, 1065353216, 0, 6, 14, 1, 1032417776, 1031127695, 990057071, 1022739087, 0, 1060487823, 1049247089, 1065353216, 0, 0, 0, 1065353216, 0, 0, 0, 1065353216, 0, 6, 14, 1, 1032417776, 990057071, 1031127695, 1022739087, -1116355953, 1059481190, 1049247089, 1065353216, 0, 0, 0, 1065353216, 0, 0, 0, 1065353216, 0, 6, 14, 1, 1032417776, 990057071, 1031127695, 1022739087, 1031127695, 1059481190, 1049247089, 1065353216, 0, 0, 0, 1065353216, 0, 0, 0, 1065353216, 0, 6, 15, 1, 1034802091, 1031127695, 1031127695, 990057071, 1050253722, 1057803469, 1047904911, 1065353216, 0, 0, 0, 1065353216, 0, 0, 0, 1065353216, 0, 6, 15, 1, 1032417776, 1031127695, 990057071, 1022739087, 1050253722, 1056629064, 1049247089, 1065353216, 0, 0, 0, 1065353216, 0, 0, 0, 1065353216, 0, 6, 15, 1, 1032417776, 1031127695, 990057071, 1022739087, 1050253722, 1058810102, 1049247089, 1065353216, 0, 0, 0, 1065353216, 0, 0, 0, 1065353216, 0, 6, 15, 1, 1032417776, 990057071, 1031127695, 1022739087, 1047904911, 1057803469, 1049247089, 1065353216, 0, 0, 0, 1065353216, 0, 0, 0, 1065353216, 0, 6, 15, 1, 1032417776, 990057071, 1031127695, 1022739087, 1052266988, 1057803469, 1049247089, 1065353216, 0, 0, 0, 1065353216, 0, 0, 0, 1065353216, 0, 6, 16, 0, 1024320445, 1017370378, 1017370378, 1017370378, 0, 0, 0, 1065353216, 0, 0, 0, 1065353216, 0, 0, 0, 1065353216, 0, 6, 17, 0, 1024320445, 1017370378, 1017370378, 1017370378, 0, 0, 0, 1065353216, 0, 0, 0, 1065353216, 0, 0, 0, 1065353216, 0, 6, 18, 0, 1024320445, 1017370378, 1017370378, 1017370378, 0, 0, 0, 1065353216, 0, 0, 0, 1065353216, 0, 0, 0, 1065353216, 0};
+alignas(16) MMX_MODEL_QUAL int MMX_geom_par[564] = {3, 0, 1065353216, 1000593162, 1017370378, 1065353216, 1063675494, 1064514355, 981668463, 1056964608, 1073741824, 0, 3, 1, 1065353216, 1000593162, 1017370378, 1065353216, 1063675494, 1064514355, 981668463, 1056964608, 1073741824, 0, 3, 2, 1065353216, 1000593162, 1017370378, 1065353216, 1063675494, 1064514355, 981668463, 1056964608, 1073741824, 941041263, 3, 3, 1065353216, 1000593162, 1017370378, 1065353216, 1063675494, 1064514355, 981668463, 1056964608, 1073741824, 966837269, 3, 4, 1065353216, 1000593162, 1017370378, 1065353216, 1063675494, 1064514355, 981668463, 1056964608, 1073741824, 1020250591, 3, 5, 1065353216, 1000593162, 1017370378, 1065353216, 1063675494, 1064514355, 981668463, 1056964608, 1073741824, 1024779564, 3, 6, 1065353216, 1000593162, 1017370378, 1065353216, 1063675494, 1064514355, 981668463, 1056964608, 1073741824, 1033117939, 3, 6, 1065353216, 1000593162, 1017370378, 1065353216, 1063675494, 1064514355, 981668463, 1056964608, 1073741824, 1033117939, 3, 6, 1065353216, 1000593162, 1017370378, 1065353216, 1063675494, 1064514355, 981668463, 1056964608, 1073741824, 1033117939, 3, 7, 1065353216, 1000593162, 1017370378, 1065353216, 1063675494, 1064514355, 981668463, 1056964608, 1073741824, 1035430532, 3, 8, 1065353216, 1000593162, 1017370378, 1065353216, 1063675494, 1064514355, 981668463, 1056964608, 1073741824, 1039061499, 3, 9, 1065353216, 1000593162, 1017370378, 1065353216, 1063675494, 1064514355, 981668463, 1056964608, 1073741824, 1038561119, 3, 10, 1065353216, 1000593162, 1017370378, 1065353216, 1063675494, 1064514355, 981668463, 1056964608, 1073741824, 1078011293, 3, 10, 1065353216, 1000593162, 1017370378, 1065353216, 1063675494, 1064514355, 981668463, 1056964608, 1073741824, 1078011293, 3, 10, 1065353216, 1000593162, 1017370378, 1065353216, 1063675494, 1064514355, 981668463, 1056964608, 1073741824, 1078011293, 3, 10, 1065353216, 1000593162, 1017370378, 1065353216, 1063675494, 1064514355, 981668463, 1056964608, 1073741824, 1078011293, 3, 10, 1065353216, 1000593162, 1017370378, 1065353216, 1063675494, 1064514355, 981668463, 1056964608, 1073741824, 1078011293, 3, 10, 1065353216, 1000593162, 1017370378, 1065353216, 1063675494, 1064514355, 981668463, 1056964608, 1073741824, 1078011293, 3, 11, 1065353216, 1000593162, 1017370378, 1065353216, 1063675494, 1064514355, 981668463, 1056964608, 1073741824, 1078011293, 3, 11, 1065353216, 1000593162, 1017370378, 1065353216, 1063675494, 1064514355, 981668463, 1056964608, 1073741824, 1078011293, 3, 11, 1065353216, 1000593162, 1017370378, 1065353216, 1063675494, 1064514355, 981668463, 1056964608, 1073741824, 1078011293, 3, 11, 1065353216, 1000593162, 1017370378, 1065353216, 1063675494, 1064514355, 981668463, 1056964608, 1073741824, 1078011293, 3, 11, 1065353216, 1000593162, 1017370378, 1065353216, 1063675494, 1064514355, 981668463, 1056964608, 1073741824, 1078011293, 3, 11, 1065353216, 1000593162, 1017370378, 1065353216, 1063675494, 1064514355, 981668463, 1056964608, 1073741824, 1078011293, 3, 12, 1065353216, 1000593162, 1017370378, 1065353216, 1063675494, 1064514355, 981668463, 1056964608, 1073741824, 0, 3, 12, 1065353216, 1000593162, 1017370378, 1065353216, 1063675494, 1064514355, 981668463, 1056964608, 1073741824, 0, 3, 12, 1065353216, 1000593162, 1017370378, 1065353216, 1063675494, 1064514355, 981668463, 1056964608, 1073741824, 0, 3, 12, 1065353216, 1000593162, 1017370378, 1065353216, 1063675494, 1064514355, 981668463, 1056964608, 1073741824, 0, 3, 12, 1065353216, 1000593162, 1017370378, 1065353216, 1063675494, 1064514355, 981668463, 1056964608, 1073741824, 0, 3, 13, 1065353216, 1000593162, 1017370378, 1065353216, 1063675494, 1064514355, 981668463, 1056964608, 1073741824, 0, 3, 13, 1065353216, 1000593162, 1017370378, 1065353216, 1063675494, 1064514355, 981668463, 1056964608, 1073741824, 0, 3, 13, 1065353216, 1000593162, 1017370378, 1065353216, 1063675494, 1064514355, 981668463, 1056964608, 1073741824, 0, 3, 13, 1065353216, 1000593162, 1017370378, 1065353216, 1063675494, 1064514355, 981668463, 1056964608, 1073741824, 0, 3, 13, 1065353216, 1000593162, 1017370378, 1065353216, 1063675494, 1064514355, 981668463, 1056964608, 1073741824, 0, 3, 14, 1065353216, 1000593162, 1017370378, 1065353216, 1063675494, 1064514355, 981668463, 1056964608, 1073741824, 0, 3, 14, 1065353216, 1000593162, 1017370378, 1065353216, 1063675494, 1064514355, 981668463, 1056964608, 1073741824, 0, 3, 14, 1065353216, 1000593162, 1017370378, 1065353216, 1063675494, 1064514355, 981668463, 1056964608, 1073741824, 0, 3, 14, 1065353216, 1000593162, 1017370378, 1065353216, 1063675494, 1064514355, 981668463, 1056964608, 1073741824, 0, 3, 14, 1065353216, 1000593162, 1017370378, 1065353216, 1063675494, 1064514355, 981668463, 1056964608, 1073741824, 0, 3, 15, 1065353216, 1000593162, 1017370378, 1065353216, 1063675494, 1064514355, 981668463, 1056964608, 1073741824, 0, 3, 15, 1065353216, 1000593162, 1017370378, 1065353216, 1063675494, 1064514355, 981668463, 1056964608, 1073741824, 0, 3, 15, 1065353216, 1000593162, 1017370378, 1065353216, 1063675494, 1064514355, 981668463, 1056964608, 1073741824, 0, 3, 15, 1065353216, 1000593162, 1017370378, 1065353216, 1063675494, 1064514355, 981668463, 1056964608, 1073741824, 0, 3, 15, 1065353216, 1000593162, 1017370378, 1065353216, 1063675494, 1064514355, 981668463, 1056964608, 1073741824, 0, 4, 16, 1073741824, 1065353216, 1017370378, 1065353216, 1063675494, 1064514355, 981668463, 1056964608, 1073741824, 1101004800, 4, 17, 1073741824, 1065353216, 1017370378, 1065353216, 1063675494, 1064514355, 981668463, 1056964608, 1073741824, 1101004800, 4, 18, 1073741824, 1065353216, 1017370378, 1065353216, 1063675494, 1064514355, 981668463, 1056964608, 1073741824, 1101004800};
 
 #define MMX_TIMESTEP 0.002
 #define MMX_GRAVITY_Z (-9.81)
diff --git a/mujoco_manip_amd/csrc/mmx_step_collision.inc b/mujoco_manip_amd/csrc/mmx_step_collision.inc
--- a/mujoco_manip_amd/csrc/mmx_step_collision.inc
+++ b/mujoco_manip_amd/csrc/mmx_step_collision.inc
@@ -121,6 +121,7 @@
     if (LANE == 0 && use_list) E.cdisp = nd;
   }
   const bool rebuild = !only_ro && !use_list;
+#if MMX_PLAIN_ROWS
   if (LANE < MMX_NGEOM) {
     const Geom G = geom_pose(E, LANE);
     float* o = gx + GXS * LANE;
@@ -133,12 +134,56 @@
     o[GX_HALF + 1] = MMX_geom_aabb[3 * LANE + 1];
     o[GX_HALF + 2] = MMX_geom_aabb[3 * LANE + 2];
   }
+#else
+  static_assert(MMX_GEOM_POSE_W == 20, "geom_pose layout");
+  int gbody = 0, gstatic = 1;
+  float grb = 0.f;
+  if (LANE < MMX_NGEOM) {
+    const int4* rp = reinterpret_cast<const int4*>(MMX_geom_pose + MMX_GEOM_POSE_W * LANE);
+    int4 w[5];
+#pragma unroll
+    for (int k = 0; k < 5; k++) w[k] = rp[k];
+    gbody = w[0].y;
+    gstatic = w[0].z;
+    grb = __int_as_float(w[0].w);
+    const int ci[12] = {w[1].w, w[2].x, w[2].y, w[2].z, w[2].w, w[3].x, w[3].y, w[3].z, w[3].w, w[4].x, w[4].y, w[4].z};
+    float cf[12];
+#pragma unroll
+    for (int k = 0; k < 12; k++) cf[k] = __int_as_float(ci[k]);
+    V3 x = V3{cf[0], cf[1], cf[2]};
+    M3 R;
+#pragma unroll
+    for (int k = 0; k < 9; k++) R.m[k] = cf[3 + k];
+    if (!gstatic) {
+      const V3 bx = body_x_moving(E, gbody);
+      const M3 bR = body_R(E, gbody);
+      x = bx + mul(bR, V3{cf[0], cf[1], cf[2]});
+      M3 Lm;
+#pragma unroll
+      for (int k = 0; k < 9; k++) Lm.m[k] = cf[3 + k];
+      R = mul(bR, Lm);
+    }
+    float* o = gx + GXS * LANE;
+    o[0] = x.x; o[1] = x.y; o[2] = x.z;
+#pragma unroll
+    for (int k = 0; k < 9; k++) o[3 + k] = R.m[k];
+    o[GX_RB] = grb;
+    o[GX_TYPE] = __int_as_float(w[0].x);
+    o[GX_HALF] = __int_as_float(w[1].x);
+    o[GX_HALF + 1] = __int_as_float(w[1].y);
+    o[GX_HALF + 2] = __int_as_float(w[1].z);
+  }
+#endif
   if (rebuild) {
     float ext = 0.f;
     if (LANE < MMX_NGEOM) {
+#if MMX_PLAIN_ROWS
       const int b = MMX_geom_body[LANE];
       if (!MMX_body_static[b]) ext = norm(V3{gx[GXS * LANE], gx[GXS * LANE + 1], gx[GXS * LANE + 2]} - body_x(E, b)) +
                                      MMX_geom_rbound[LANE];
+#else
+      if (!gstatic) ext = norm(V3{gx[GXS * LANE], gx[GXS * LANE + 1], gx[GXS * LANE + 2]} - body_x_moving(E, gbody)) + grb;
+#endif
     }
     ext = wave_max(ext);
     if (LANE == 0) E.crad = ext;
@@ -223,6 +268,7 @@
   constexpr int NCP = (COL_LIST + WG - 1) / WG;
   int ce[NCP];
   int ncls[3] = {0, 0, 0};
+  unsigned long long cm0[3] = {0ull, 0ull, 0ull};
 #pragma unroll
   for (int q = 0; q < NCP; q++) {
     const int k = q * WG + LANE;
@@ -237,11 +283,22 @@
         else if (obb_overlap(A, B, geom_half(gx, g1), geom_half(gx, g2))) c = (A.type == GT_BOX && B.type == GT_BOX) ? 1 : 2;
       }
 #pragma unroll
-      for (int t = 0; t < 3; t++) ncls[t] += __popcll(__ballot(c == t));
+      for (int t = 0; t < 3; t++) {
+        const unsigned long long m = __ballot(c == t);
+        if (q == 0) cm0[t] = m;
+        ncls[t] += __popcll(m);
+      }
     }
     ce[q] = p | (c << 24);
   }
   SYNC();
+  if (!MMX_PLAIN_ROWS && nc <= WG) {
+    const int c = ce[0] >> 24;
+    const unsigned long long m = c == 0 ? cm0[0] : (c == 1 ? cm0[1] : cm0[2]);
+    const int pos = (c == 0 ? 0 : (c == 1 ? ncls[0] : ncls[0] + ncls[1])) +
+                    (int)__builtin_amdgcn_mbcnt_hi((unsigned)(m >> 32), __builtin_amdgcn_mbcnt_lo((unsigned)m, 0u));
+    if (c < 3) cand[pos] = ce[0] & 0xFFFFFF;
+  } else {
   int base[3] = {0, ncls[0], ncls[0] + ncls[1]};
 #pragma unroll
   for (int q = 0; q < NCP; q++) {
@@ -250,6 +307,7 @@
 #pragma unroll
       for (int t = 0; t < 3; t++) base[t] = wave_compact(c == t, cand, base[t], ce[q] & 0xFFFFFF);
     }
+  }
   }
   if (LANE == 0) {
     E.ncls[0] = ncls[0];
@@ -334,6 +392,36 @@
   float* stats = E.stats;
   CLK_DECL;
   float* scr = scr_of(E);
+#if !MMX_PLAIN_ROWS
+  static_assert(MMX_MAXCON == WG && MMX_MAXCON % 16 == 0, "one contact per lane, keys in batches of 16");
+  const int n = __builtin_amdgcn_readfirstlane(min(E.ncon, MMX_MAXCON));
+  const int4* keys = reinterpret_cast<const int4*>(con_of(E) + CL_KEY * MMX_MAXCON);
+  const int key = con_key(crec(E, LANE)) & 0xFFFF;
+  int rank = 0;
+#pragma unroll
+  for (int j0 = 0; j0 < MMX_MAXCON; j0 += 16) {
+    if (j0 >= n) break;
+    int4 kq[4];
+#pragma unroll
+    for (int q = 0; q < 4; q++) kq[q] = keys[j0 / 4 + q];
+#pragma unroll
+    for (int q = 0; q < 4; q++) {
+      const int kk[4] = {kq[q].x, kq[q].y, kq[q].z, kq[q].w};
+#pragma unroll
+      for (int t = 0; t < 4; t++) rank += (j0 + 4 * q + t < n) & ((kk[t] & 0xFFFF) < key);
+    }
+  }
+  if (LANE < n) {
+    float rec[CL_F];
+#pragma unroll
+    for (int f = 0; f < CL_F; f++) rec[f] = con_of(E)[f * MMX_MAXCON + LANE];
+#pragma unroll
+    for (int f = 0; f < CL_F; f++) con_of(E)[f * MMX_MAXCON + rank] = rec[f];
+  }
+  if (LANE == 0) E.ncon = n;
+  SYNC();
+  (void)scr;
+#else
   const int n = min(E.ncon, MMX_MAXCON);
   float* tmp = scr + COL_WORK;
   int kb = 0, rank = 0;
@@ -348,6 +436,7 @@
   for (int k = LANE; k < MMX_MAXCON * CL_F; k += WG) con_of(E)[k] = tmp[k];
   if (LANE == 0) E.ncon = n;
   SYNC();
+#endif
   PROBE(5, stats, STAT_T_AUX3);
 }
 
diff --git a/mujoco_manip_amd/csrc/mmx_step_constraints.inc b/mujoco_manip_amd/csrc/mmx_step_constraints.inc
--- a/mujoco_manip_amd/csrc/mmx_step_constraints.inc
+++ b/mujoco_manip_amd/csrc/mmx_step_constraints.inc
@@ -49,50 +49,113 @@
   P.idiag = P.dim > 1 ? 2.f * P.mu0 * P.mu0 * (it + P.mu0 * P.mu0 * it) : it;
   return P;
 }
+struct GeomPar {
+  int condim, body;
+  float fr0, fr1, solref[2], solimp[5], invw;
+};
+static_assert(MMX_GEOM_PAR_W == 12, "geom_par layout");
+DEV GeomPar geom_par(int g) {
+  const int4* r = reinterpret_cast<const int4*>(MMX_geom_par + MMX_GEOM_PAR_W * g);
+  const int4 a = r[0], b = r[1], c = r[2];
+  GeomPar G;
+  G.condim = a.x;
+  G.body = a.y;
+  G.fr0 = __int_as_float(a.z);
+  G.fr1 = __int_as_float(a.w);
+  G.solref[0] = __int_as_float(b.x);
+  G.solref[1] = __int_as_float(b.y);
+  G.solimp[0] = __int_as_float(b.z);
+  G.solimp[1] = __int_as_float(b.w);
+  G.solimp[2] = __int_as_float(c.x);
+  G.solimp[3] = __int_as_float(c.y);
+  G.solimp[4] = __int_as_float(c.z);
+  G.invw = __int_as_float(c.w);
+  return G;
+}
+DEV ConPar contact_params(float dist, const GeomPar& G1, const GeomPar& G2) {
+  ConPar P;
+  P.dim = max(G1.condim, G2.condim);
+  P.mu0 = fmaxf(G1.fr0, G2.fr0);
+  P.mu1 = fmaxf(G1.fr1, G2.fr1);
+  float solref[2], solimp[5];
+#pragma unroll
+  for (int k = 0; k < 2; k++) solref[k] = 0.5f * (G1.solref[k] + G2.solref[k]);
+#pragma unroll
+  for (int k = 0; k < 5; k++) solimp[k] = 0.5f * (G1.solimp[k] + G2.solimp[k]);
+  float impr;
+  row_ref(solref, solimp, dist, impr, P.kid, P.B);
+  const float tran = G1.invw + G2.invw;
+  const float it = impr * tran;
+  P.idiag = P.dim > 1 ? 2.f * P.mu0 * P.mu0 * (it + P.mu0 * P.mu0 * it) : it;
+  return P;
+}
 DEV V3 contact_t1(V3 n) {
   const V3 y = (n.y < 0.5f && n.y > -0.5f) ? V3{0.f, 1.f, 0.f} : V3{0.f, 0.f, 1.f};
   return normalize(y - n * dot(n, y));
 }
 
-DEV float contact_row(EnvSh& E, int row, const CReg& cc, int rr, const ConPar& P) {
+DEV int body_word(int b1, int b2, int dim) {
+  return (body_block(b1) + 1) | ((body_block(b2) + 1) << 3) | ((int)anc_mask(b1) << 6) | ((int)anc_mask(b2) << 15) | (dim << 24);
+}
+DEV int body_word_dim(int bw) { return bw >> 24; }
+DEV bool body_word_arm(int bw) { return ((bw >> 6) & 0x3FFFF) != 0; }
+DEV float contact_row(EnvSh& E, int row, const CReg& cc, int rr, const ConPar& P, int bw, bool any_arm) {
   const V3 p = V3{cc[CL_POS], cc[CL_POS + 1], cc[CL_POS + 2]};
   const V3 n = V3{cc[CL_N], cc[CL_N + 1], cc[CL_N + 2]};
+#if MMX_PLAIN_ROWS
   const int b1 = MMX_geom_body[con_g1(cc)], b2 = MMX_geom_body[con_g2(cc)];
+  const int k1 = body_block(b1), k2 = body_block(b2);
+  const unsigned am1 = anc_mask(b1), am2 = anc_mask(b2);
+#else
+  const int k1 = (bw & 7) - 1, k2 = ((bw >> 3) & 7) - 1;
+  const unsigned am1 = (bw >> 6) & 0x1FFu, am2 = (bw >> 15) & 0x1FFu;
+#endif
   const int dim = P.dim;
   const bool used = rr == 0 || (rr < 3 && dim >= 3) || (rr == 3 && dim >= 4);
   const V3 t1 = contact_t1(n);
   const V3 u = rr == 0 ? n : (rr == 1 ? t1 : (rr == 2 ? cross(n, t1) : V3{0.f, 0.f, 0.f}));
   const V3 w = rr == 3 ? n : V3{0.f, 0.f, 0.f};
   const float idiag = P.idiag;
-  const int k1 = body_block(b1), k2 = body_block(b2);
   int rb0 = k1 >= 0 ? k1 : k2, rb1 = (k1 >= 0 && k2 >= 0 && k2 != k1) ? k2 : BLK_NONE;
   if (rb1 != BLK_NONE && rb1 < rb0) {
     const int t = rb0;
     rb0 = rb1;
     rb1 = t;
   }
-  const unsigned am1 = anc_mask(b1), am2 = anc_mask(b2);
   float vel = 0.f;
   float arm[9];
-  const V3 pu = cross(p, u) + w;
-#pragma unroll
-  for (int d = 0; d < 9; d++) {
-    const float coef = (float)((int)((am2 >> d) & 1u) - (int)((am1 >> d) & 1u));
-    const SV sd = load_S(E, d);
-    arm[d] = coef * (dot(u, sd.v) + dot(sd.w, pu));
-    vel = fmaf(arm[d], E.qvel[d], vel);
+#pragma unroll
+  for (int d = 0; d < 9; d++) arm[d] = 0.f;
+  if (any_arm) {
+    const V3 pu = cross(p, u) + w;
+#pragma unroll
+    for (int d = 0; d < 9; d++) {
+      const float coef = (float)((int)((am2 >> d) & 1u) - (int)((am1 >> d) & 1u));
+      const SV sd = load_S(E, d);
+      arm[d] = coef * (dot(u, sd.v) + dot(sd.w, pu));
+      vel = fmaf(arm[d], E.qvel[d], vel);
+    }
   }
   float cubeA[6], cubeB[6];
   float cvs[2][6];
 #pragma unroll
   for (int side = 0; side < 2; side++) {
-    const int b = side ? b2 : b1, blk = side ? k2 : k1;
+    const int blk = side ? k2 : k1;
 #pragma unroll
     for (int j = 0; j < 6; j++) cvs[side][j] = 0.f;
     if (blk > 0) {
       const float sg = side ? 1.f : -1.f;
+#if MMX_PLAIN_ROWS
+      const int b = side ? b2 : b1;
       const V3 x = body_x(E, b);
       const M3 R = body_R(E, b);
+#else
+      const int s = 10 + blk;
+      const V3 x = V3{E.bx[s][0], E.bx[s][1], E.bx[s][2]};
+      M3 R;
+#pragma unroll
+      for (int k = 0; k < 9; k++) R.m[k] = E.bR[s][k];
+#endif
       cvs[side][0] = sg * u.x;
       cvs[side][1] = sg * u.y;
       cvs[side][2] = sg * u.z;
@@ -141,11 +204,24 @@
     hi_act = MMX_jnt_range[2 * LANE + 1] - q < 0.f;
     nlim = (int)lo_act + (int)hi_act;
   }
+  int bword = 0;
+#if !MMX_PLAIN_ROWS
+  GeomPar gp1{}, gp2{};
+#endif
   if (LANE < ncon) {
     const int g1 = con_g1(own), g2 = con_g2(own);
+#if MMX_PLAIN_ROWS
     const int dim = max(MMX_geom_condim[g1], MMX_geom_condim[g2]);
+    const int cb1 = MMX_geom_body[g1], cb2 = MMX_geom_body[g2];
+#else
+    gp1 = geom_par(g1);
+    gp2 = geom_par(g2);
+    const int dim = max(gp1.condim, gp2.condim);
+    const int cb1 = gp1.body, cb2 = gp2.body;
+    bword = body_word(cb1, cb2, dim);
+#endif
     nedge = dim == 1 ? 1 : 2 * (dim - 1);
-    const int k1 = body_block(MMX_geom_body[g1]), k2 = body_block(MMX_geom_body[g2]);
+    const int k1 = body_block(cb1), k2 = body_block(cb2);
     int rb0 = k1 >= 0 ? k1 : k2, rb1 = (k1 >= 0 && k2 >= 0 && k2 != k1) ? k2 : BLK_NONE;
     if (rb1 != BLK_NONE && rb1 < rb0) {
       const int t = rb0;
@@ -191,7 +267,11 @@
   }
   PROBE(3, stats, STAT_T_AUX1);
   ConPar Pc{1, 0.f, 0.f, 0.f, 0.f, 1.f};
+#if MMX_PLAIN_ROWS
   if (LANE < ncon) Pc = contact_params(own);
+#else
+  if (LANE < ncon) Pc = contact_params(own[CL_DIST], gp1, gp2);
+#endif
   if (LANE < ncon) {
 #pragma unroll
     for (int rr = 0; rr < 4; rr++)
@@ -210,7 +290,15 @@
     const int m = r < nefc ? __float_as_int(dget(E, r)) : -1;
     const int c = m >= 0 ? (m & 255) : 0;
     ConPar P;
+#if MMX_PLAIN_ROWS
+    const int bw = 0;
+    const bool any_arm = true;
     P.dim = __shfl(Pc.dim, c);
+#else
+    const int bw = __shfl(bword, c);
+    const bool any_arm = __ballot(m >= 0 && body_word_arm(bw)) != 0ull;
+    P.dim = body_word_dim(bw);
+#endif
     P.mu0 = __shfl(Pc.mu0, c);
     P.mu1 = __shfl(Pc.mu1, c);
     P.kid = __shfl(Pc.kid, c);
@@ -220,7 +308,7 @@
     cc.v[CL_DIST] = 0.f;
 #pragma unroll
     for (int k = CL_POS; k < CL_F; k++) cc.v[k] = __shfl(own.v[k], c);
-    if (m >= 0) mu[q] = contact_row(E, r, cc, m >> 8, P);
+    if (m >= 0) mu[q] = contact_row(E, r, cc, m >> 8, P, bw, any_arm);
   }
   row = arow;
   float jv[16];
diff --git a/mujoco_manip_amd/csrc/mmx_step_lds.inc b/mujoco_manip_amd/csrc/mmx_step_lds.inc
--- a/mujoco_manip_amd/csrc/mmx_step_lds.inc
+++ b/mujoco_manip_amd/csrc/mmx_step_lds.inc
@@ -117,6 +117,9 @@
 #define DELAY_HELPER() do { } while (0)
 #define DELAY_ENV() do { } while (0)
 #endif
+#ifndef MMX_PLAIN_ROWS
+#define MMX_PLAIN_ROWS 0
+#endif
 DEV float* scr_of(EnvSh& E) { return reinterpret_cast<float*>(&E.J); }
 DEV const float* scr_of(const EnvSh& E) { return reinterpret_cast<const float*>(&E.J); }
 DEV float* obs_of(EnvSh& E) { return scr_of(E) + SCR_OBS; }
@@ -217,6 +220,10 @@
   const int s = body_slot(b);
   return V3{E.bx[s][0], E.bx[s][1], E.bx[s][2]};
 }
+DEV V3 body_x_moving(const EnvSh& E, int b) {
+  const int s = body_slot(b);
+  return V3{E.bx[s][0], E.bx[s][1], E.bx[s][2]};
+}
 DEV M3 body_R(const EnvSh& E, int b) {
   M3 R;
   const int s = body_slot(b);
```

Result: no change. 3.510 million, median of 2 (-0.1%).
